# Strong-AI-Lab/ct-vae

Measured on AMD Instinct MI355X. Metric: images/sec/GPU fwd+bwd, 64×64×3 bs=64; recon+KL vs CPU ref, higher is better.
Workload: dtype f32; 1 GPU; VanillaVAE 64x64x3 train step fwd+loss+bwd+Adam (configs/vae.yaml shapes at the batch BASELINE.json's metric names, bs=64, on one MI355X; BASELINE.json configs[1..4] are the `configs` entries); per_gpu_batch=64, global_batch=64, latent_dim=128, parallelism=single, hipgraph=True, allreduce_overlap=False

## Files before the change

ct-vae_amd/csrc/api.hip:

```cpp
#include "../../include/ctvae_hip.h"

#include "common.hpp"
#include "gatlayer.hpp"
#include "glinear.hpp"
#include "pair.hpp"

namespace ctvae {
int launch_tapgemm(const ConvGeom& g, const float* G, const float* W, const float* bias, const float* add,
                   const float* mask, int mask_act, float* S, int act, float* bn_part, float* ws, size_t ws_floats,
                   hipStream_t st, const BnBwdFuse* bnb = nullptr, const InXform* xf = nullptr,
                   const WinoFilters* wf = nullptr, SplitKRaw* raw = nullptr, int out_pix = 0);
bool out_pix_supported(const ConvGeom& g, size_t ws_floats, int out_pix);
bool wino_supported(const ConvGeom& g, size_t ws_floats);
bool wino_enabled();
int wino_set_enabled(int on);
int launch_crop_resize_u8(const unsigned char* img, const long long* rows, float* out, int B, int N, int H, int W, int crop,
                          int S, hipStream_t st);
bool thin_forward_supported(const ConvGeom& g);
bool thin_wgrad_supported(const ConvGeom& g);
int tapgemm_bnb_rows(const ConvGeom& g, size_t ws_floats);
bool img_dgrad_supported(const ConvGeom& g);
void tapgemm_plan(const ConvGeom& g, size_t ws_floats, TapGemmPlan& p);
int launch_wgrad(const ConvGeom& g, const float* X, const float* dY, float* dW, float* dbias, float* ws, size_t ws_bytes,
                 int accumulate, hipStream_t st, const InXform* xf = nullptr, const DyXform* dyx = nullptr);
int launch_bn_forward(const float* y, int R, int C, const float* gamma, const float* beta, float* running_mean,
                      float* running_var, float momentum, float eps, int training, int act, float* out, float* save_mean,
                      float* save_invstd, float* ws, size_t ws_bytes, long long* nbt, hipStream_t st,
                      float* coef_out = nullptr);
int launch_bn_finish_forward(const float* y, int R, int C, int nparts, const float* gamma, const float* beta,
                             float* running_mean, float* running_var, float momentum, float eps, int training, int act,
                             float* out, float* save_mean, float* save_invstd, float* ws, long long* nbt, hipStream_t st,
                             float* coef_out = nullptr, const float* mean_base = nullptr);
size_t bn_workspace_floats(int C, int nparts);
int launch_bn_backward(const float* ga, const float* beta, const float* y, int R, int C, const float* gamma,
                       const float* save_mean, const float* save_invstd, int act, float* gy, float* dgamma, float* dbeta,
                       int accumulate, float* ws, size_t ws_bytes, const float* part_in, int part_rows, hipStream_t st,
                       float* coef_out = nullptr, const float* coef_in = nullptr);
int launch_wino_filters_batch(int n, const float* const* W, float* const* Uf, float* const* Ub, const int* Ci, const int* Co,
                              hipStream_t st);
bool upconv_wgrad_supported(const ConvGeom& g);
bool img_enc_supported(const ConvGeom& g);
bool img_conv_supported(const ConvGeom& g);
int launch_img_backward_fused(const ConvGeom& g, const float* dY, const float* W, float* dX, const BnBwdFuse* bnb, float* ws,
                              float** part_out, float** pbias_out, int* nparts, bool want_bias, hipStream_t st);
size_t img_backward_fused_ws_floats(const ConvGeom& g);
int wgrad_finish_slabs(const float* part, float* dW, long n, int nparts, const float* pbias, float* dbias, long nb, int accumulate,
                       hipStream_t st);
int launch_permute(const float* in, float* out, int B, int C, int P, int to_nhwc, hipStream_t st);
int launch_gat_score(int mode, const float* xl, const float* xr, const float* attr, const float* we, const float* att, float* out,
                     int B, int N, int H, int C, float slope, hipStream_t st);
int launch_gat_score_backward(const float* xl, const float* xr, const float* attr, const float* we, const float* att,
                              const float* g, float* dxl, float* dxr, float* datt_part, float* dwe_part, int B, int N, int H,
                              int C, float slope, hipStream_t st);
int launch_gauss_latent_fwd(float* heads, const float* eps_in, const unsigned long long* rng, float* eps_out, float* z, int B,
                            int L, hipStream_t st, const float* slices, int S, const float* bias);
int launch_splitk_permute(const float* slices, int S, float* out, int B, int C, int P, hipStream_t st);
int launch_gauss_latent_bwd(const float* g_mu, const float* g_lv, const float* g_z, const float* heads, const float* eps,
                            float* g_heads, unsigned long long* rng_bump, int B, int L, hipStream_t st, int gz_slices);
int launch_ct_reg_forward(const float* adj, const float* graph, const float* uni, float* part, float ckl, float cgs, float cpt,
                          int B, int N, hipStream_t st);
int launch_ct_reg_backward(const float* adj, const float* graph, const float* uni, const float* part, const float* g_loss,
                           float ckl, float cgs, float cpt, float* d_adj, float* d_graph, int B, int N, hipStream_t st);
int launch_ct_blend_softmax_forward(const float* y, const float* mask, float* probs, long R, int Hs, int D, hipStream_t st);
int launch_ct_blend_softmax_backward(const float* g, const float* probs, const float* y, const float* mask, float* dy, float* dmask,
                                     long R, int Hs, int D, hipStream_t st);
int launch_ct_latent_ce_forward(const float* probs, const long long* target, float* row_loss, long R, int D, hipStream_t st);
int launch_ct_latent_ce_backward(const float* probs, const long long* target, const float* g_loss, float* d_probs, long R, int D,
                                 hipStream_t st);
int launch_ct_mask_forward(const float* x, const float* action, const float* pe, const float* keep, float scale, const float* W,
                           const float* bias, const float* expo, int B, int S, int D, int A, float* inter, float* p, float* sample,
                           float* soft, hipStream_t st);
int launch_ct_mask_backward(const float* x, const float* action, const float* pe, const float* keep, float scale,
                            const float* inter, const float* p, const float* soft, const float* g, int B, int S, int D, int A,
                            float* dWp, float* dbp, hipStream_t st);
int launch_ladder_forward(const float* mu_e, const float* lv_e, const float* mu_t, const float* lv_t, const float* eps, int B, int D,
                          float* z, float* kl, hipStream_t st);
int launch_ladder_backward(const float* gz, const float* gkl, const float* mu_e, const float* lv_e, const float* mu_t, const float* lv_t,
                           const float* eps, int B, int D, float* g_mu_e, float* g_lv_e, float* g_mu_t, float* g_lv_t, hipStream_t st);
int launch_gamma_reparam_forward(const float* alpha, const float* beta, const float* zhat, float shape_b, float* z, long n, hipStream_t st);
int launch_gamma_reparam_backward(const float* g, const float* alpha, const float* beta, const float* zhat, float shape_b, float* ga,
                                  float* gb, long n, hipStream_t st);
int launch_gamma_kl_forward(const float* alpha, const float* beta, int B, int D, float prior_alpha, float prior_beta, float* out,
                            float* ws, size_t ws_bytes, hipStream_t st);
int launch_gamma_kl_backward(const float* g, const float* alpha, const float* beta, int B, int D, float prior_alpha, float prior_beta,
                             float* ga, float* gb, hipStream_t st);
int launch_sigmoid(const float* x_or_g, const float* y, float* out, long n, int backward, hipStream_t st);
int launch_tc_forward(const float* z, const float* mu, const float* lv, const float* liw, int B, int D, float* out3, float* lse_s,
                      float* lse_d, float* ws, size_t ws_bytes, hipStream_t st);
int launch_tc_backward(const float* z, const float* mu, const float* lv, const float* liw, const float* lse_s, const float* lse_d,
                       const float* g3, int B, int D, float* dz, float* dmu, float* dlv, hipStream_t st);
int launch_vamp_forward(const float* z, const float* mu, const float* lv, const float* pmu, const float* plv, int B, int D, int K,
                        float* out3, float* wgt, float* ws, size_t ws_bytes, hipStream_t st);
int launch_vamp_backward(const float* z, const float* mu, const float* lv, const float* pmu, const float* plv, const float* wgt,
                         const float* g, int B, int D, int K, float* dz, float* dmu, float* dlv, float* dpmu, float* dplv,
                         hipStream_t st);
int launch_swd_forward(const float* z, const float* prior, const float* proj, int N, int D, int S, float p, float weight, float* out,
                       float* grad_z, float* ws, size_t ws_bytes, hipStream_t st);
int launch_ct_blend_forward(const float* s0, const float* s1, const float* mask, float* out, long rows, hipStream_t st);
int launch_ct_blend_backward(const float* g, const float* s0, const float* s1, const float* mask, float* g0, float* g1, float* gm,
                             long rows, hipStream_t st);
int launch_group_rowsum(const float* parts, long mat_stride, int nmat, int rows, int C, int ld, const int* grp, int G, float* out,
                        int accumulate, hipStream_t st);
int launch_ct_posenc_forward(const float* x, const float* pe, const float* keep, float scale, float* out, long n, int sd,
                             hipStream_t st);
int launch_ct_posenc_backward(const float* g, const float* keep, float scale, float* gx, long n, hipStream_t st);
int launch_one_hot(const long long* inds, long n, int N, float* out, hipStream_t st);
int launch_ct_sample_forward(const float* p, const float* expo, float* out, float* soft, float* weighted, long n, hipStream_t st);
int launch_ct_sample_backward(const float* gs, const float* gw, const float* p, const float* soft, const float* sample, float* gp,
                              long n, hipStream_t st);
int launch_pair_mlp_forward(const float* u, const float* v, int ld, const float* w2, const float* b2, float* out, int B, int N,
                            int H, float slope, int per_sample, const int* row_of, hipStream_t st);
int launch_pair_mlp_backward(const float* u, const float* v, int ld, const float* w2, const float* out, const float* g_out,
                             float* dU, float* dV, int ldd, float* dw2_part, float* db2_part, int B, int N, int H, float slope,
                             int per_sample, const int* row_of, hipStream_t st);
int launch_act_bwd(const float* gout, const float* out, float* gin, long n, int act, hipStream_t st);
int launch_act_fwd(const float* in, float* out, long n, int act, hipStream_t st);
int launch_reparam_fwd(const float* mu, long mu_rs, const float* lv, long lv_rs, const float* eps, float* z, int B, int L,
                       hipStream_t st);
int launch_reparam_bwd(const float* gz, const float* lv, long lv_rs, const float* eps, float* gmu, float* glv, int B, int L,
                       hipStream_t st);
int launch_adam(float* p, const float* g, float* m, float* v, float* state, long n, float grad_scale, hipStream_t st);
size_t adam_state_floats();
int launch_adam_clipped(float* p, const float* g, float* m, float* v, float* state, long n, float grad_scale, int algorithm,
                        float clip, float* ws, float* norm_out, hipStream_t st);
size_t grad_clip_workspace_floats();
int launch_adam_mark_members(int* hits, int nhits, const int* group, int B, hipStream_t st);
int launch_adam_block_flags(const int* present, const int* hit_index, int* hits, int nhits, const float* bstate, int* active,
                            int nb, int until_first, hipStream_t st);
int launch_adam_block_flags_local(const int* present, const int* hit_index, int* hits, int nhits, int* active, int nb,
                                  hipStream_t st);
int launch_adam_block_flags_finish(const float* bstate, int* active, int nb, int until_first, hipStream_t st);
int launch_adam_blocks(float* p, const float* g, float* m, float* v, float* state, long n, float grad_scale, int algorithm,
                       float clip, float* ws, float* norm_out, const int* blk_lo, const int* blk_hi, float* bstate,
                       const int* active, int nb, hipStream_t st);
int launch_ssim_forward(const float* a, const float* b, const float* window, float* part, float* loss, float* coef, int B, int C, int H,
                        int W, const float* weights, hipStream_t st);
int launch_ssim_backward(const float* a, const float* b, const float* window, const float* coef, const float* g_loss, float* g_a, int B,
                         int C, int H, int W, hipStream_t st);
float* defer_wgrad_ws(float* ws, size_t ws_floats);
void defer_wgrad_done();
int defer_begin(float* arena, size_t arena_floats);
int defer_flush(hipStream_t st);
int launch_gumbel_fwd(const float* p, const float* noise, float* out, float* soft, long n, hipStream_t st);
int launch_gumbel_bwd(const float* go, const float* p, const float* soft, float* gp, long n, hipStream_t st);
int launch_gumbel_softmax_fwd(const float* z, const float* u, float* s, long rows, int Q, float temp, float eps, hipStream_t st);
int launch_gumbel_softmax_bwd(const float* gs, const float* s, float* gz, long rows, int Q, float temp, hipStream_t st);
int launch_cat_kl_fwd(const float* logits, long rows, int Q, int B, float eps, float c, float* out, float* ws, size_t ws_bytes,
                      hipStream_t st);
int launch_cat_kl_bwd(const float* logits, const float* go, float* gq, long rows, int Q, int B, float eps, float c, hipStream_t st);
int launch_iw_loss_forward(const float* recons, const float* x, long n, int R, int rep, const float* mu, const float* lv, int L,
                           int S, float M_N, float* lp, float* kld, float* coef, float* out4, hipStream_t st);
int launch_iw_loss_backward(const float* recons, const float* x, long n, int R, int rep, const float* mu, const float* lv, int L,
                            float M_N, const float* coef, const float* go, float* g_recons, float* g_mu, float* g_lv,
                            hipStream_t st);
int launch_mmd_forward(const float* z, const float* p, int N, int D, int kind, float c, float eps, float w_pp, float w_zz,
                       float w_pz, float* out4, float* grad, float* ws, size_t ws_bytes, hipStream_t st);
size_t dip_state_floats(int B, int D);
int launch_dip_forward(const float* mu, long mu_rs, const float* lv, long lv_rs, int B, int D, float l_diag, float l_off,
                       float* state, hipStream_t st);
int launch_dip_backward(const float* state, const float* go, float* g_mu, float* g_lv, int B, int D, hipStream_t st);
int launch_column_moments(const float* z, int N, int L, float* mean, float* var, float* mn, float* mx, hipStream_t st);
int launch_mi_matrix(const float* z, const float* lo, const float* hi, const int32_t* factors, const int32_t* sizes, int N, int L,
                     int F, float* mi, uint8_t* bins, hipStream_t st);
int launch_group_var_argmin(const float* z, const float* gvar, const uint8_t* active, int G, int B, int L, int32_t* arg, float* val,
                            hipStream_t st);
int launch_image_grid_u8(const float* x, long sN, long sC, long sH, long sW, int N, int C, int H, int W, int nrow, int pad,
                         int normalize, int has_range, float lo, float hi, float pad_value, int scanlines, uint8_t* out,
                         size_t out_bytes, float* ws, size_t ws_bytes, hipStream_t st);
int launch_image_grid_each_u8(const float* x, long sN, long sC, long sH, long sW, int N, int C, int H, int W, int nrow, int pad,
                              int normalize, int has_range, float lo, float hi, float pad_value, int scanlines, uint8_t* out,
                              size_t out_bytes, float* ws, size_t ws_bytes, hipStream_t st);
int launch_action_hits(const float* probas, const float* action, int N, int A, int* counts, hipStream_t st);
int launch_loss_forward(const float* r, const float* x, long n, const float* mu, long mu_rs, const float* lv, long lv_rs,
                        int B, int L, float M_N, const float* extra, float* out4, float* ws, size_t ws_bytes,
                        hipStream_t st, float logcosh_alpha, float* g_r = nullptr, float* g_mu = nullptr, float* g_lv = nullptr,
                        int ract = 0);
int launch_mse_backward(const float* r, const float* x, const float* go, float* gr, long n, hipStream_t st, float logcosh_alpha,
                        int ract = 0);
int launch_loss_backward(const float* r, const float* x, const float* go, float* gr, long n, float logcosh_alpha, const float* mu,
                         long mu_rs, const float* lv, long lv_rs, float* gmu, float* glv, int B, int L, float M_N, hipStream_t st,
                         int ract = 0);
int launch_kl_backward(const float* mu, long mu_rs, const float* lv, long lv_rs, const float* go, float* gmu, float* glv,
                       int B, int L, float M_N, hipStream_t st);
int launch_vq_inds(const float* lat, const float* cb, long long* inds, int B, int HW, int D, int K, int C, hipStream_t st);
int launch_vq_lookup(const float* lat, const float* cb, const long long* inds, float* out, float* vq_loss, float beta, int B,
                     int HW, int D, int K, int C, float* ws, size_t ws_bytes, hipStream_t st);
int launch_vq_backward(const float* gq, const float* gvq, const float* lat, const float* cb, const long long* inds,
                       float* glat, float* dcb, int accumulate, float beta, int B, int HW, int D, int K, int C, float* ws, size_t ws_bytes,
                       hipStream_t st);
}

using namespace ctvae;

static bool conv_kind_ok(int kind) {
  const int base = kind & ~CTVAE_W_CI_TAP;
  return base == CTVAE_CONV || (base == CTVAE_CONVT && !(kind & CTVAE_W_CI_TAP));
}
static int conv_geom(ConvGeom& g, int kind, int gkind0, int B, int H, int W, int Ci, int Co, int k, int stride, int pad, int out_pad) {
  const int rc = build_geom(g, gkind0 + ((kind & ~CTVAE_W_CI_TAP) == CTVAE_CONV ? 0 : 1), B, H, W, Ci, Co, k, stride, pad, out_pad);
  if (rc) return rc;
  if (kind & CTVAE_W_CI_TAP) {
    g.wts = Co;
    g.wrs = k * k * Co;
  }
  return 0;
}

extern "C" {

const char* ctvae_version(void) { return "0.1.0"; }
const char* ctvae_arch(void) { return "gfx950"; }

const char* ctvae_error_string(int code) {
  if (code == 0) return "success";
  if (code == kErrBadArg) return "ctvae: unsupported shape or bad argument";
  if (code == kErrWorkspace) return "ctvae: workspace too small";
  if (code > 0) return hipGetErrorString((hipError_t)code);
  return "ctvae: unknown error";
}

int ctvae_crop_resize_u8(const uint8_t* images, const int64_t* rows, float* out, int B, int N, int H, int W, int crop, int size,
                         void* stream) {
  if (!images || !rows || !out) return kErrBadArg;
  return launch_crop_resize_u8(images, (const long long*)rows, out, B, N, H, W, crop, size, (hipStream_t)stream);
}

int ctvae_winograd_enable(int on) { return wino_set_enabled(on); }

size_t ctvae_workspace_bytes(void) { return (size_t)256 << 20; }

int ctvae_conv_forward(int kind, const float* x, const float* w, const float* bias, const float* add, float* y, int B,
                       int H, int W, int Ci, int Co, int k, int stride, int pad, int out_pad, int act, const float* in_scale,
                       const float* in_shift, int in_act, float* wino_dgrad_filters_out, const float* wino_fwd_filters, float* ws,
                       size_t ws_bytes, void* stream) {
  if (!x || !w || !y || !conv_kind_ok(kind)) return kErrBadArg;
  if ((in_scale != nullptr) != (in_shift != nullptr)) return kErrBadArg;
  ConvGeom g;
  if (conv_geom(g, kind, 0, B, H, W, Ci, Co, k, stride, pad, out_pad)) return kErrBadArg;
  if ((wino_dgrad_filters_out != nullptr || wino_fwd_filters != nullptr) &&
      !ctvae_conv_wino_filter_floats(kind, B, H, W, Ci, Co, k, stride, pad, out_pad, ws_bytes))
    return kErrBadArg;
  const InXform xf{in_scale, in_shift, in_act};
  const WinoFilters wf{wino_fwd_filters, wino_fwd_filters != nullptr ? nullptr : wino_dgrad_filters_out};
  return launch_tapgemm(g, x, w, bias, add, nullptr, 0, y, act, nullptr, ws, ws_bytes / sizeof(float), (hipStream_t)stream,
                        nullptr, &xf, &wf);
}

int ctvae_linear_pixmajor_supported(int B, int Ci, int C, int P, size_t ws_bytes) {
  ConvGeom g;
  if (B <= 0 || Ci <= 0 || C <= 0 || P <= 1 || conv_geom(g, CTVAE_CONV, 0, B, 1, 1, Ci, C * P, 1, 1, 0, 0)) return 0;
  return out_pix_supported(g, ws_bytes / sizeof(float), P) ? 1 : 0;
}

int ctvae_linear_pixmajor_forward(const float* x, const float* w, const float* bias, float* y, int B, int Ci, int C, int P, int act,
                                  float* ws, size_t ws_bytes, void* stream) {
  if (!x || !w || !y || !ctvae_linear_pixmajor_supported(B, Ci, C, P, ws_bytes)) return kErrBadArg;
  ConvGeom g;
  if (conv_geom(g, CTVAE_CONV, 0, B, 1, 1, Ci, C * P, 1, 1, 0, 0)) return kErrBadArg;
  return launch_tapgemm(g, x, w, bias, nullptr, nullptr, 0, y, act, nullptr, ws, ws_bytes / sizeof(float), (hipStream_t)stream,
                        nullptr, nullptr, nullptr, nullptr, P);
}

int ctvae_wino_filters_batch(int n, const float* const* w, float* const* fwd_filters, float* const* dgrad_filters, const int* Ci,
                             const int* Co, void* stream) {
  return launch_wino_filters_batch(n, w, fwd_filters, dgrad_filters, Ci, Co, (hipStream_t)stream);
}

size_t ctvae_conv_wino_filter_floats(int kind, int B, int H, int W, int Ci, int Co, int k, int stride, int pad, int out_pad,
                                     size_t ws_bytes) {
  if (kind != CTVAE_CONV || !wino_enabled()) return 0;
  ConvGeom gf, gb;
  if (build_geom(gf, 0, B, H, W, Ci, Co, k, stride, pad, out_pad) || build_geom(gb, 2, B, H, W, Ci, Co, k, stride, pad, out_pad))
    return 0;
  const size_t wsf = ws_bytes / sizeof(float);
  return (wino_supported(gf, wsf) && wino_supported(gb, wsf)) ? (size_t)16 * Ci * Co : 0;
}

int ctvae_conv_input_transform_supported(int kind, int B, int H, int W, int Ci, int Co, int k, int stride, int pad,
                                         int out_pad) {
  if (!conv_kind_ok(kind)) return 0;
  ConvGeom g;
  if (conv_geom(g, kind, 0, B, H, W, Ci, Co, k, stride, pad, out_pad)) return 0;
  if (thin_forward_supported(g) && thin_wgrad_supported(g)) return 1;
  if (upconv_wgrad_supported(g)) return 1;
  if (img_enc_supported(g) || img_conv_supported(g)) return 0;
  if (wino_enabled() && wino_supported(g, (size_t)1 << 26)) return 0;
  TapGemmPlan pl;
  tapgemm_plan(g, (size_t)1 << 26, pl);
  if (pl.thin || pl.BM == 0) return 0;
  return ((g.gC % KC) == 0 && (g.sC % 4) == 0 && g.wT == 0) ? 1 : 0;
}

int ctvae_conv_bn_act_apply_is_separate(int kind, int B, int H, int W, int Ci, int Co, int k, int stride, int pad, int out_pad,
                                        size_t ws_bytes) {
  if (!conv_kind_ok(kind)) return 0;
  ConvGeom g;
  if (conv_geom(g, kind, 0, B, H, W, Ci, Co, k, stride, pad, out_pad)) return 0;
  TapGemmPlan plan;
  tapgemm_plan(g, ws_bytes / sizeof(float), plan);
  return (plan.splitk > 1 && bn_fused_ok(g.B * g.sH * g.sW, Co)) ? 0 : 1;
}

int ctvae_conv_bn_act_forward(int kind, const float* x, const float* w, const float* bias, const float* gamma,
                              const float* beta, float* running_mean, float* running_var, float momentum, float eps,
                              int training, int act, float* y, float* a_out, float* save_mean, float* save_invstd,
                              float* scale_shift_out, int64_t* num_batches_tracked, int B, int H, int W, int Ci, int Co, int k,
                              int stride, int pad, int out_pad, const float* in_scale, const float* in_shift, int in_act,
                              float* ws, size_t ws_bytes, void* stream) {
  long long* nbt = (long long*)num_batches_tracked;
  if (!x || !w || !gamma || !beta || !y || !ws || !conv_kind_ok(kind)) return kErrBadArg;
  if ((in_scale != nullptr) != (in_shift != nullptr)) return kErrBadArg;
  if (in_scale != nullptr && !ctvae_conv_input_transform_supported(kind, B, H, W, Ci, Co, k, stride, pad, out_pad)) return kErrBadArg;
  const InXform xf{in_scale, in_shift, in_act};
  const InXform* xfp = in_scale != nullptr ? &xf : nullptr;
  if (!a_out && !scale_shift_out) return kErrBadArg;
  if (training && (!save_mean || !save_invstd)) return kErrBadArg;
  if (!training && (!running_mean || !running_var)) return kErrBadArg;
  if (Co % 4 != 0) return kErrBadArg;
  ConvGeom g;
  if (conv_geom(g, kind, 0, B, H, W, Ci, Co, k, stride, pad, out_pad)) return kErrBadArg;
  const size_t wsf = ws_bytes / sizeof(float);
  TapGemmPlan plan;
  tapgemm_plan(g, wsf, plan);
  const int R = g.B * g.sH * g.sW;
  if (plan.splitk > 1 || !training) {
    SplitKRaw raw{ws, 0};
    const bool fused = training && plan.splitk > 1 && bn_fused_ok(R, Co);
    int rc = launch_tapgemm(g, x, w, bias, nullptr, nullptr, 0, y, ACT_NONE, nullptr, ws, wsf, (hipStream_t)stream, nullptr, xfp,
                            nullptr, fused ? &raw : nullptr);
    if (rc) return rc;
    if (raw.splitk > 1) {
      const BnFusedFwd p{ws, row_map_of(g), raw.splitk, R, Co, bias, gamma, beta, running_mean, running_var, momentum, eps, save_mean, save_invstd,
                         scale_shift_out, nbt, y, a_out, act};
      return launch_bn_fused_forward(p, (hipStream_t)stream);
    }
    return launch_bn_forward(y, R, Co, gamma, beta, running_mean, running_var, momentum, eps, training, act, a_out, save_mean,
                             save_invstd, ws, ws_bytes, nbt, (hipStream_t)stream, scale_shift_out);
  }
  const int nparts = plan.bn_parts;
  if (wsf < bn_workspace_floats(Co, nparts)) return kErrWorkspace;
  int rc = launch_tapgemm(g, x, w, bias, nullptr, nullptr, 0, y, ACT_NONE, ws, nullptr, 0, (hipStream_t)stream, nullptr, xfp);
  if (rc) return rc;
  return launch_bn_finish_forward(y, R, Co, nparts, gamma, beta, running_mean, running_var, momentum, eps, training, act,
                                  a_out, save_mean, save_invstd, ws, nbt, (hipStream_t)stream, scale_shift_out);
}

int ctvae_conv_dgrad(int kind, const float* dy, const float* w, const float* add, const float* mask, int mask_act,
                     float* dx, int B, int H, int W, int Ci, int Co, int k, int stride, int pad, int out_pad,
                     const float* wino_filters, float* ws, size_t ws_bytes, void* stream) {
  if (!dy || !w || !dx || !conv_kind_ok(kind)) return kErrBadArg;
  ConvGeom g;
  if (conv_geom(g, kind, 2, B, H, W, Ci, Co, k, stride, pad, out_pad)) return kErrBadArg;
  if (wino_filters != nullptr && !ctvae_conv_wino_filter_floats(kind, B, H, W, Ci, Co, k, stride, pad, out_pad, ws_bytes))
    return kErrBadArg;
  const WinoFilters wf{wino_filters, nullptr};
  return launch_tapgemm(g, dy, w, nullptr, add, mask, mask_act, dx, ACT_NONE, nullptr, ws, ws_bytes / sizeof(float),
                        (hipStream_t)stream, nullptr, nullptr, &wf);
}

int ctvae_conv_wgrad(int kind, const float* x, const float* dy, float* dw, float* dbias, int B, int H, int W, int Ci,
                     int Co, int k, int stride, int pad, int out_pad, int accumulate, const float* in_scale,
                     const float* in_shift, int in_act, const float* dy_bn_y, const float* dy_bn_coef, int dy_bn_act,
                     float* gy_out, float* bn_dgamma, float* bn_dbeta, int bn_accumulate, float* ws, size_t ws_bytes,
                     void* stream) {
  if (!x || !dy || !dw || !ws || !conv_kind_ok(kind)) return kErrBadArg;
  if ((in_scale != nullptr) != (in_shift != nullptr)) return kErrBadArg;
  if ((dy_bn_y != nullptr) != (dy_bn_coef != nullptr) || (gy_out != nullptr && dy_bn_y == nullptr)) return kErrBadArg;
  if ((bn_dgamma != nullptr) != (bn_dbeta != nullptr) || (bn_dgamma != nullptr && (dy_bn_y == nullptr || gy_out != nullptr)))
    return kErrBadArg;
  ConvGeom g;
  if (conv_geom(g, kind, 0, B, H, W, Ci, Co, k, stride, pad, out_pad)) return kErrBadArg;
  const InXform xf{in_scale, in_shift, in_act};
  const DyXform dyx{dy_bn_y, dy_bn_coef, gy_out, dy_bn_act, bn_dgamma, bn_dbeta, bn_accumulate};
  float* wws = defer_wgrad_ws(ws, ws_bytes / sizeof(float));
  const int rc = launch_wgrad(g, x, dy, dw, dbias, wws, ws_bytes, accumulate, (hipStream_t)stream, &xf, &dyx);
  defer_wgrad_done();
  return rc;
}

int ctvae_defer_begin(float* arena, size_t arena_bytes) { return defer_begin(arena, arena_bytes / sizeof(float)); }
int ctvae_defer_flush(void* stream) { return defer_flush((hipStream_t)stream); }

int ctvae_conv_backward_bn_rows(int kind, int B, int H, int W, int Ci, int Co, int k, int stride, int pad, int out_pad,
                                size_t ws_bytes) {
  if (!conv_kind_ok(kind)) return 0;
  ConvGeom g;
  if (conv_geom(g, kind, 2, B, H, W, Ci, Co, k, stride, pad, out_pad)) return 0;
  PairCtx ctx;
  pair_ctx() = &ctx;
  const int rows = tapgemm_bnb_rows(g, ((ws_bytes / 2) & ~(size_t)255) / sizeof(float));
  pair_ctx() = nullptr;
  return rows;
}

static thread_local int g_lazy_pixel_major = 0;

static int conv_backward_impl(int kind, const float* x, const float* dy, const float* w, float* dw, float* dbias, float* dx, int B,
                        int H, int W, int Ci, int Co, int k, int stride, int pad, int out_pad, int accumulate, const float* mask,
                        int mask_act, const float* wino_filters, const float* bn_y, const float* bn_mean,
                        const float* bn_invstd, const float* bn_gamma, const float* bn_beta, int bn_act, float* bn_part,
                        int bn_part_rows, float* bn_coef_out, float* bn_dgamma, float* bn_dbeta, int bn_accumulate,
                        const float* in_scale, const float* in_shift, int in_act,
                        const float* dy_bn_y, const float* dy_bn_coef, int dy_bn_act, float* gy_out, float* ws, size_t ws_bytes,
                        void* stream, float* dx_slices) {
  if (!x || !dy || !w || !dw || (!dx && !dx_slices) || !ws || !conv_kind_ok(kind)) return kErrBadArg;
  const bool bn = bn_part != nullptr;
  if (bn_coef_out != nullptr && !bn) return kErrBadArg;
  if ((bn_dgamma != nullptr) != (bn_dbeta != nullptr) || (bn_dgamma != nullptr && bn_coef_out == nullptr)) return kErrBadArg;
  if ((in_scale != nullptr) != (in_shift != nullptr)) return kErrBadArg;
  if ((dy_bn_y != nullptr) != (dy_bn_coef != nullptr) || (dy_bn_y != nullptr) != (gy_out != nullptr)) return kErrBadArg;
  if (bn && (!bn_y || !bn_mean || !bn_invstd || !bn_gamma || !bn_beta)) return kErrBadArg;
  ConvGeom gw, gd;
  if (conv_geom(gw, kind, 0, B, H, W, Ci, Co, k, stride, pad, out_pad)) return kErrBadArg;
  if (conv_geom(gd, kind, 2, B, H, W, Ci, Co, k, stride, pad, out_pad)) return kErrBadArg;
  const size_t half_bytes = (ws_bytes / 2) & ~(size_t)255, half_floats = half_bytes / sizeof(float);
  float* ws_d = ws + half_floats;
  if (wino_filters != nullptr && !ctvae_conv_wino_filter_floats(kind, B, H, W, Ci, Co, k, stride, pad, out_pad, half_bytes))
    return kErrBadArg;
  const hipStream_t st = (hipStream_t)stream;
  PairCtx ctx;
  pair_ctx() = &ctx;
  if (bn) {
    const int rows = tapgemm_bnb_rows(gd, half_floats);
    if (rows <= 0 || rows != bn_part_rows || (img_dgrad_supported(gd) && mask != nullptr)) {
      pair_ctx() = nullptr;
      return kErrBadArg;
    }
  }
  {
    TapGemmPlan pl;
    tapgemm_plan(gd, half_floats, pl);
    ctx.dgrad_wgs = (long)pl.mtiles * pl.ntiles * gd.ncls * (pl.splitk > 1 ? pl.splitk : 1);
    int kmax = 0;
    for (int c = 0; c < gd.ncls; ++c) kmax = gd.ntaps[c] * gd.gC / KC > kmax ? gd.ntaps[c] * gd.gC / KC : kmax;
    ctx.dgrad_chunks = pl.splitk > 1 ? (kmax + pl.splitk - 1) / pl.splitk : kmax;
  }
  const InXform xf{in_scale, in_shift, in_act};
  const DyXform dyx{dy_bn_y, dy_bn_coef, gy_out, dy_bn_act};
  int rc;
  if (bn && bn_act != ACT_TANH && x == bn_y && in_scale != nullptr && in_act == bn_act && mask == nullptr && dy_bn_y == nullptr &&
      img_conv_supported(gw) && img_dgrad_supported(gd) && img_backward_fused_ws_floats(gd) <= half_floats) {
    float *part = nullptr, *pb = nullptr;
    int np = 0;
    const BnBwdFuse f{bn_y, bn_mean, bn_invstd, bn_gamma, bn_beta, bn_act, bn_part};
    rc = launch_img_backward_fused(gd, dy, w, dx, &f, ws, &part, &pb, &np, dbias != nullptr, st);
    if (!rc) rc = wgrad_finish_slabs(part, dw, 9L * 32 * 3, np, pb, dbias, 3L, accumulate, st);
  } else {
    float* wws = bn_coef_out == nullptr ? defer_wgrad_ws(ws, half_floats) : ws;
    rc = launch_wgrad(gw, x, dy, dw, dbias, wws, half_bytes, accumulate, st, &xf, &dyx);
    defer_wgrad_done();
    if (!rc) {
    const WinoFilters wf{wino_filters, nullptr};
    const BnBwdFuse f{bn_y, bn_mean, bn_invstd, bn_gamma, bn_beta, bn_act, bn_part};
      SplitKRaw raw{dx_slices, 0, g_lazy_pixel_major};
      g_lazy_pixel_major = 0;
      rc = launch_tapgemm(gd, gy_out != nullptr ? gy_out : dy, w, nullptr, nullptr, mask, mask_act, dx, ACT_NONE, nullptr, ws_d,
                          half_floats, st, bn ? &f : nullptr, nullptr, &wf, dx_slices != nullptr ? &raw : nullptr);
      if (!rc && dx_slices != nullptr && raw.splitk <= 1) rc = kErrBadArg;
    }
  }
  pair_ctx() = nullptr;
  if (rc) return rc;
  if (bn_coef_out != nullptr) {
    ctx.haveBF = true;
    ctx.bf = BnFinJob{bn_part, bn_part_rows, Ci, (float)((long)B * H * W), bn_gamma, bn_mean, bn_invstd, bn_beta, bn_coef_out,
                      bn_dgamma, bn_dbeta, bn_accumulate};
  }
  return pair_flush(ctx, st);
}

int ctvae_conv_backward(int kind, const float* x, const float* dy, const float* w, float* dw, float* dbias, float* dx, int B,
                        int H, int W, int Ci, int Co, int k, int stride, int pad, int out_pad, int accumulate, const float* mask,
                        int mask_act, const float* wino_filters, const float* bn_y, const float* bn_mean,
                        const float* bn_invstd, const float* bn_gamma, const float* bn_beta, int bn_act, float* bn_part,
                        int bn_part_rows, float* bn_coef_out, float* bn_dgamma, float* bn_dbeta, int bn_accumulate,
                        const float* in_scale, const float* in_shift, int in_act,
                        const float* dy_bn_y, const float* dy_bn_coef, int dy_bn_act, float* gy_out, float* ws, size_t ws_bytes,
                        void* stream) {
  return conv_backward_impl(kind, x, dy, w, dw, dbias, dx, B, H, W, Ci, Co, k, stride, pad, out_pad, accumulate, mask, mask_act,
                            wino_filters, bn_y, bn_mean, bn_invstd, bn_gamma, bn_beta, bn_act, bn_part, bn_part_rows, bn_coef_out,
                            bn_dgamma, bn_dbeta, bn_accumulate, in_scale, in_shift, in_act, dy_bn_y, dy_bn_coef, dy_bn_act, gy_out, ws,
                            ws_bytes, stream, nullptr);
}

int ctvae_conv_backward_lazy_slices(int kind, int B, int H, int W, int Ci, int Co, int k, int stride, int pad, int out_pad,
                                    int for_bn, size_t ws_bytes) {
  if (!conv_kind_ok(kind)) return 0;
  ConvGeom g;
  if (conv_geom(g, kind, 2, B, H, W, Ci, Co, k, stride, pad, out_pad)) return 0;
  const size_t half_floats = ((ws_bytes / 2) & ~(size_t)255) / sizeof(float);
  if (img_dgrad_supported(g) || (wino_enabled() && wino_supported(g, half_floats))) return 0;
  PairCtx ctx;
  pair_ctx() = &ctx;
  TapGemmPlan pl;
  tapgemm_plan(g, half_floats, pl);
  pair_ctx() = nullptr;
  const long Mc = (long)g.B * g.Qh * g.Qw;
  if (pl.thin || pl.splitk <= 1) return 0;
  if (for_bn && (Mc % 4 != 0 || !bn_fused_ok(B * H * W, Ci))) return 0;
  return pl.splitk;
}

int ctvae_conv_backward_lazy(int kind, const float* x, const float* dy, const float* w, float* dw, float* dbias, float* dx_slices,
                             int B, int H, int W, int Ci, int Co, int k, int stride, int pad, int out_pad, int accumulate,
                             const float* in_scale, const float* in_shift, int in_act, int pixel_major, float* ws, size_t ws_bytes,
                             void* stream) {
  if (!dx_slices) return kErrBadArg;
  g_lazy_pixel_major = pixel_major;
  return conv_backward_impl(kind, x, dy, w, dw, dbias, nullptr, B, H, W, Ci, Co, k, stride, pad, out_pad, accumulate, nullptr, 0,
                            nullptr, nullptr, nullptr, nullptr, nullptr, nullptr, 0, nullptr, 0, nullptr, nullptr, nullptr, 0, in_scale,
                            in_shift, in_act, nullptr, nullptr, 0, nullptr, ws, ws_bytes, stream, dx_slices);
}

int ctvae_bn_backward_fused(const float* g_a_slices, int slices, int kind, int B, int H, int W, int Ci, int Co, int k, int stride,
                            int pad, int out_pad, const float* y, const float* gamma, const float* beta, const float* save_mean,
                            const float* save_invstd, int act, float* g_y, float* dgamma, float* dbeta, int accumulate, void* stream) {
  if (!g_a_slices || slices < 1 || !y || !gamma || !beta || !save_mean || !save_invstd || !g_y || !dgamma || !dbeta) return kErrBadArg;
  if (!conv_kind_ok(kind)) return kErrBadArg;
  ConvGeom g;
  if (conv_geom(g, kind, 2, B, H, W, Ci, Co, k, stride, pad, out_pad)) return kErrBadArg;
  const BnFusedBwd p{g_a_slices, row_map_of(g), slices, B * H * W, Ci, y, gamma, beta, save_mean, save_invstd, act, g_y, dgamma,
                     dbeta, accumulate};
  return launch_bn_fused_backward(p, (hipStream_t)stream);
}

int ctvae_conv_wgrad_bn_apply_supported(int kind, int B, int H, int W, int Ci, int Co, int k, int stride, int pad, int out_pad) {
  if (!conv_kind_ok(kind)) return 0;
  ConvGeom g;
  if (conv_geom(g, kind, 0, B, H, W, Ci, Co, k, stride, pad, out_pad)) return 0;
  if (upconv_wgrad_supported(g)) return 1;
  return img_enc_supported(g) ? 2 : 0;
}

int ctvae_bn_forward(const float* y, int R, int C, const float* gamma, const float* beta, float* running_mean,
                     float* running_var, float momentum, float eps, int training, int act, float* out,
                     float* save_mean, float* save_invstd, int64_t* num_batches_tracked, float* ws, size_t ws_bytes,
                     void* stream) {
  if (!y || !gamma || !beta || !out || !ws) return kErrBadArg;
  if (training && (!save_mean || !save_invstd)) return kErrBadArg;
  if (!training && (!running_mean || !running_var)) return kErrBadArg;
  return launch_bn_forward(y, R, C, gamma, beta, running_mean, running_var, momentum, eps, training, act, out, save_mean,
                           save_invstd, ws, ws_bytes, (long long*)num_batches_tracked, (hipStream_t)stream);
}

int ctvae_bn_backward(const float* g_a, const float* beta, const float* y, int R, int C, const float* gamma,
                      const float* save_mean, const float* save_invstd, int act, float* g_y, float* dgamma,
                      float* dbeta, int accumulate, const float* part_in, int part_rows, float* coef_out,
                      const float* coef_in, float* ws, size_t ws_bytes, void* stream) {
  if (!g_a || !beta || !y || !gamma || !save_mean || !save_invstd || !dgamma || !dbeta || !ws) return kErrBadArg;
  if (!g_y && !coef_out) return kErrBadArg;
  if ((part_in != nullptr) != (part_rows > 0)) return kErrBadArg;
  if (coef_in != nullptr && (!g_y || part_in != nullptr || coef_out != nullptr)) return kErrBadArg;
  return launch_bn_backward(g_a, beta, y, R, C, gamma, save_mean, save_invstd, act, g_y, dgamma, dbeta, accumulate, ws,
                            ws_bytes, part_in, part_rows, (hipStream_t)stream, coef_out, coef_in);
}

int ctvae_gat_score(int mode, const float* xl, const float* xr, const float* attr, const float* we, const float* att, float* out,
                    int B, int N, int H, int C, float slope, void* stream) {
  if (!xl || !xr || !attr || !we || !att || !out || (mode != 0 && mode != 1)) return kErrBadArg;
  return launch_gat_score(mode, xl, xr, attr, we, att, out, B, N, H, C, slope, (hipStream_t)stream);
}

int ctvae_gat_score_backward(const float* xl, const float* xr, const float* attr, const float* we, const float* att,
                             const float* g, float* d_xl, float* d_xr, float* d_att_part, float* d_we_part, int B, int N, int H,
                             int C, float slope, void* stream) {
  if (!xl || !xr || !attr || !we || !att || !g || !d_xl || !d_xr || !d_att_part || !d_we_part) return kErrBadArg;
  return launch_gat_score_backward(xl, xr, attr, we, att, g, d_xl, d_xr, d_att_part, d_we_part, B, N, H, C, slope,
                                   (hipStream_t)stream);
}

int ctvae_gat_layer_forward(const float* xl, const float* xr, int ld, const float* adj, const float* we, const float* att,
                            const float* bias, const int32_t* head_map, float* out, int ldo, float* alpha, int B, int Hs, int C,
                            float slope, int act, void* stream) {
  const GatLayerArgs a{xl, xr, ld, adj, we, att, bias, head_map, out, ldo, alpha, B, Hs, C, slope, act};
  return launch_gat_layer_forward(a, (hipStream_t)stream);
}

int ctvae_gat_layer_backward(const float* xl, const float* xr, int ld, const float* adj, const float* we, const float* att,
                             const float* bias, const int32_t* head_map, const float* out, int ldo, const float* alpha,
                             const float* g_out, float* dS, float* dattr, float* d_xl, float* d_xr, int ldd, float* d_bias_part,
                             float* d_att_part, float* d_we_part, float* d_adj, int accumulate_dadj, int B, int Hs, int C,
                             float slope, int act, void* stream) {
  GatBwdArgs p{};
  p.f = GatLayerArgs{xl, xr, ld, adj, we, att, bias, head_map, const_cast<float*>(out), ldo, const_cast<float*>(alpha), B, Hs, C,
                     slope, act};
  p.g_out = g_out; p.dS = dS; p.dattr = dattr; p.dxl = d_xl; p.dxr = d_xr; p.ldd = ldd;
  p.dbias_part = d_bias_part; p.datt_part = d_att_part; p.dwe_part = d_we_part;
  return launch_gat_layer_backward(p, d_adj, accumulate_dadj, (hipStream_t)stream);
}

int ctvae_gauss_latent_forward(float* heads, const float* eps_in, const uint64_t* rng, float* eps_out, float* z, int B, int L,
                               const float* head_slices, int slices, const float* head_bias, void* stream) {
  return launch_gauss_latent_fwd(heads, eps_in, (const unsigned long long*)rng, eps_out, z, B, L, (hipStream_t)stream, head_slices,
                                 slices, head_bias);
}

int ctvae_gauss_latent_backward(const float* g_mu, const float* g_logvar, const float* g_z, const float* heads, const float* eps,
                                float* g_heads, uint64_t* rng_bump, int B, int L, int g_z_slices, void* stream) {
  return launch_gauss_latent_bwd(g_mu, g_logvar, g_z, heads, eps, g_heads, (unsigned long long*)rng_bump, B, L, (hipStream_t)stream,
                                 g_z_slices);
}

int ctvae_splitk_permute(const float* slices, int n_slices, float* out, int B, int C, int P, void* stream) {
  return launch_splitk_permute(slices, n_slices, out, B, C, P, (hipStream_t)stream);
}

int ctvae_conv_forward_lazy_slices(int kind, int B, int H, int W, int Ci, int Co, int k, int stride, int pad, int out_pad,
                                   size_t ws_bytes) {
  if (!conv_kind_ok(kind)) return 0;
  ConvGeom g;
  if (conv_geom(g, kind, 0, B, H, W, Ci, Co, k, stride, pad, out_pad)) return 0;
  const size_t wsf = ws_bytes / sizeof(float);
  if (img_enc_supported(g) || img_conv_supported(g) || upconv_wgrad_supported(g) || (wino_enabled() && wino_supported(g, wsf))) return 0;
  TapGemmPlan pl;
  tapgemm_plan(g, wsf, pl);
  return (pl.thin || pl.splitk <= 1) ? 0 : pl.splitk;
}

int ctvae_conv_forward_lazy(int kind, const float* x, const float* w, float* y_slices, int B, int H, int W, int Ci, int Co, int k,
                            int stride, int pad, int out_pad, float* ws, size_t ws_bytes, void* stream) {
  if (!x || !w || !y_slices || !ws || !conv_kind_ok(kind)) return kErrBadArg;
  ConvGeom g;
  if (conv_geom(g, kind, 0, B, H, W, Ci, Co, k, stride, pad, out_pad)) return kErrBadArg;
  SplitKRaw raw{y_slices, 0, 1};
  const int rc = launch_tapgemm(g, x, w, nullptr, nullptr, nullptr, 0, nullptr, ACT_NONE, nullptr, ws, ws_bytes / sizeof(float),
                                (hipStream_t)stream, nullptr, nullptr, nullptr, &raw);
  if (rc) return rc;
  return raw.splitk > 1 ? 0 : kErrBadArg;
}

int ctvae_ct_reg_forward(const float* adj, const float* graph, const float* uniform, float* part4, float ckl, float cgs, float cpt,
                         int B, int N, void* stream) {
  return launch_ct_reg_forward(adj, graph, uniform, part4, ckl, cgs, cpt, B, N, (hipStream_t)stream);
}

int ctvae_ct_reg_backward(const float* adj, const float* graph, const float* uniform, const float* part4, const float* g_loss,
                          float ckl, float cgs, float cpt, float* d_adj, float* d_graph, int B, int N, void* stream) {
  return launch_ct_reg_backward(adj, graph, uniform, part4, g_loss, ckl, cgs, cpt, d_adj, d_graph, B, N, (hipStream_t)stream);
}

int ctvae_ct_blend_softmax_forward(const float* y, const float* mask, float* probs, long R, int Hs, int D, void* stream) {
  return launch_ct_blend_softmax_forward(y, mask, probs, R, Hs, D, (hipStream_t)stream);
}

int ctvae_ct_blend_softmax_backward(const float* g, const float* probs, const float* y, const float* mask, float* dy, float* dmask,
                                    long R, int Hs, int D, void* stream) {
  return launch_ct_blend_softmax_backward(g, probs, y, mask, dy, dmask, R, Hs, D, (hipStream_t)stream);
}

int ctvae_ct_latent_ce_forward(const float* probs, const int64_t* target, float* row_loss, long R, int D, void* stream) {
  return launch_ct_latent_ce_forward(probs, (const long long*)target, row_loss, R, D, (hipStream_t)stream);
}

int ctvae_ct_latent_ce_backward(const float* probs, const int64_t* target, const float* g_loss, float* d_probs, long R, int D,
                                void* stream) {
  return launch_ct_latent_ce_backward(probs, (const long long*)target, g_loss, d_probs, R, D, (hipStream_t)stream);
}

int ctvae_ct_mask_forward(const float* x, const float* action, const float* pe, const float* keep, float scale, const float* W,
                          const float* bias, const float* expo, int B, int S, int D, int A, float* inter, float* p, float* sample,
                          float* soft, void* stream) {
  return launch_ct_mask_forward(x, action, pe, keep, scale, W, bias, expo, B, S, D, A, inter, p, sample, soft, (hipStream_t)stream);
}

int ctvae_ct_mask_backward(const float* x, const float* action, const float* pe, const float* keep, float scale, const float* inter,
                           const float* p, const float* soft, const float* g, int B, int S, int D, int A, float* dWp, float* dbp,
                           void* stream) {
  return launch_ct_mask_backward(x, action, pe, keep, scale, inter, p, soft, g, B, S, D, A, dWp, dbp, (hipStream_t)stream);
}

int ctvae_ct_sample_forward(const float* p, const float* expo, float* sample, float* soft, float* weighted, long n, void* stream) {
  return launch_ct_sample_forward(p, expo, sample, soft, weighted, n, (hipStream_t)stream);
}

int ctvae_ct_sample_backward(const float* g_sample, const float* g_weighted, const float* p, const float* soft, const float* sample,
                             float* g_p, long n, void* stream) {
  return launch_ct_sample_backward(g_sample, g_weighted, p, soft, sample, g_p, n, (hipStream_t)stream);
}

int ctvae_ct_blend_forward(const float* s0, const float* s1, const float* mask, float* out, long rows, void* stream) {
  return launch_ct_blend_forward(s0, s1, mask, out, rows, (hipStream_t)stream);
}

int ctvae_ct_blend_backward(const float* g, const float* s0, const float* s1, const float* mask, float* g0, float* g1, float* g_mask,
                            long rows, void* stream) {
  return launch_ct_blend_backward(g, s0, s1, mask, g0, g1, g_mask, rows, (hipStream_t)stream);
}

int ctvae_ct_posenc_forward(const float* x, const float* pe, const float* keep, float scale, float* out, long n, int sd,
                            void* stream) {
  return launch_ct_posenc_forward(x, pe, keep, scale, out, n, sd, (hipStream_t)stream);
}

int ctvae_ct_posenc_backward(const float* g, const float* keep, float scale, float* g_x, long n, void* stream) {
  return launch_ct_posenc_backward(g, keep, scale, g_x, n, (hipStream_t)stream);
}

int ctvae_one_hot(const int64_t* inds, long n, int N, float* out, void* stream) {
  return launch_one_hot((const long long*)inds, n, N, out, (hipStream_t)stream);
}

int ctvae_group_rowsum(const float* parts, long mat_stride, int nmat, int rows, int C, int ld, const int32_t* group, int G, float* out,
                       int accumulate, void* stream) {
  return launch_group_rowsum(parts, mat_stride, nmat, rows, C, ld, group, G, out, accumulate, (hipStream_t)stream);
}

static int glin_fill(GLinArgs& a, int nseg, int N, const float* const* W, const int* ldw, const int64_t* w_gstride,
                     const float* const* bias, const int* b_gstride, const int32_t* const* group) {
  if (nseg < 1 || nseg > kGLinMaxSeg || !W || !ldw || !w_gstride) return kErrBadArg;
  a.nseg = nseg;
  a.N = N;
  for (int s = 0; s < nseg; ++s) {
    a.W[s] = W[s];
    a.ldw[s] = ldw[s];
    a.wgs[s] = (long)w_gstride[s];
    a.bias[s] = bias ? bias[s] : nullptr;
    a.bgs[s] = b_gstride ? b_gstride[s] : 0;
    a.group[s] = group ? group[s] : nullptr;
  }
  return 0;
}

int ctvae_glinear_forward(const float* x, int ldx, int K, int nseg, int N, const float* const* W, const int* ldw,
                          const int64_t* w_gstride, const float* const* bias, const int* b_gstride,
                          const int32_t* const* group, float* y, int ldy, int B, void* stream) {
  GLinArgs a{};
  if (int rc = glin_fill(a, nseg, N, W, ldw, w_gstride, bias, b_gstride, group)) return rc;
  a.x = x; a.ldx = ldx; a.K = K; a.y = y; a.ldy = ldy; a.B = B;
  return launch_glinear_forward(a, (hipStream_t)stream);
}

int ctvae_glinear_dgrad(const float* dy, int ldy, int nseg, int N, const float* const* W, const int* ldw,
                        const int64_t* w_gstride, const int32_t* const* group, float* dx, int ldx, int K, int B, void* stream) {
  GLinArgs a{};
  if (int rc = glin_fill(a, nseg, N, W, ldw, w_gstride, nullptr, nullptr, group)) return rc;
  a.x = nullptr; a.ldx = ldx; a.K = K; a.y = const_cast<float*>(dy); a.ldy = ldy; a.B = B;
  return launch_glinear_dgrad(a, dx, (hipStream_t)stream);
}

size_t ctvae_glinear_wgrad_ws_bytes(int G, int N, int K, int B, int grouped) {
  if (G <= 0 || N <= 0 || K <= 0 || B <= 0) return 0;
  return glinear_wgrad_ws_floats(G, N, K, glinear_wgrad_slices(B, G, grouped != 0)) * sizeof(float);
}

int ctvae_glinear_wgrad(const float* x, int ldx, int K, const float* dy, int ldy, int col0, int N, const int32_t* group, int G,
                        int B, float* dW, int ldo, float* dbias, int accumulate, float* ws, size_t ws_bytes, void* stream) {
  return launch_glinear_wgrad(x, ldx, K, dy, ldy, col0, N, group, G, B, dW, ldo, dbias, accumulate, ws, ws_bytes / sizeof(float),
                              (hipStream_t)stream);
}

int ctvae_pair_mlp_forward(const float* u, const float* v, int ld, const float* w2, const float* b2, float* out, int B, int N,
                           int H, float slope, int per_sample, const int32_t* row_of, void* stream) {
  if (!u || !v || !w2 || !out) return kErrBadArg;
  return launch_pair_mlp_forward(u, v, ld, w2, b2, out, B, N, H, slope, per_sample, row_of, (hipStream_t)stream);
}

int ctvae_pair_mlp_backward(const float* u, const float* v, int ld, const float* w2, const float* out, const float* g_out,
                            float* d_u, float* d_v, int ldd, float* d_w2_part, float* d_b2_part, int B, int N, int H, float slope,
                            int per_sample, const int32_t* row_of, void* stream) {
  if (!u || !v || !w2 || !out || !g_out || !d_u || !d_v || !d_w2_part || !d_b2_part) return kErrBadArg;
  return launch_pair_mlp_backward(u, v, ld, w2, out, g_out, d_u, d_v, ldd, d_w2_part, d_b2_part, B, N, H, slope, per_sample,
                                  row_of, (hipStream_t)stream);
}

int ctvae_permute(const float* in, float* out, int B, int C, int P, int to_nhwc, void* stream) {
  if (!in || !out || B <= 0 || C <= 0 || P <= 0) return kErrBadArg;
  return launch_permute(in, out, B, C, P, to_nhwc, (hipStream_t)stream);
}

int ctvae_act_forward(const float* in, float* out, long n, int act, void* stream) {
  if (!in || !out || n <= 0) return kErrBadArg;
  return launch_act_fwd(in, out, n, act, (hipStream_t)stream);
}

int ctvae_act_backward(const float* g_out, const float* out, float* g_in, long n, int act, void* stream) {
  if (!g_out || !out || !g_in || n <= 0) return kErrBadArg;
  return launch_act_bwd(g_out, out, g_in, n, act, (hipStream_t)stream);
}

int ctvae_reparam_forward(const float* mu, long mu_rs, const float* logvar, long lv_rs, const float* eps, float* z, int B,
                          int L, void* stream) {
  if (!mu || !logvar || !eps || !z || B <= 0 || L <= 0) return kErrBadArg;
  return launch_reparam_fwd(mu, mu_rs, logvar, lv_rs, eps, z, B, L, (hipStream_t)stream);
}

int ctvae_reparam_backward(const float* g_z, const float* logvar, long lv_rs, const float* eps, float* g_mu,
                           float* g_logvar, int B, int L, void* stream) {
  if (!g_z || !logvar || !eps || !g_mu || !g_logvar || B <= 0 || L <= 0) return kErrBadArg;
  return launch_reparam_bwd(g_z, logvar, lv_rs, eps, g_mu, g_logvar, B, L, (hipStream_t)stream);
}

int ctvae_loss_forward(const float* recons, const float* x, long n, const float* mu, long mu_rs, const float* logvar,
                       long lv_rs, int B, int L, float M_N, const float* extra, float* out4, float* ws, size_t ws_bytes,
                       void* stream) {
  if (!recons || !x || !out4 || !ws || n <= 0) return kErrBadArg;
  if ((mu == nullptr) != (logvar == nullptr)) return kErrBadArg;
  return launch_loss_forward(recons, x, n, mu, mu_rs, logvar, lv_rs, B, L, M_N, extra, out4, ws, ws_bytes,
                             (hipStream_t)stream, 0.f);
}

int ctvae_loss_forward_grad(const float* recons, const float* x, long n, const float* mu, long mu_rs, const float* logvar,
                            long lv_rs, int B, int L, float M_N, const float* extra, float* out4, float* g_recons, float* g_mu,
                            float* g_logvar, int recons_act, float* ws, size_t ws_bytes, void* stream) {
  if (!recons || !x || !out4 || !ws || n <= 0 || !mu || !logvar || !g_recons || !g_mu || !g_logvar) return kErrBadArg;
  return launch_loss_forward(recons, x, n, mu, mu_rs, logvar, lv_rs, B, L, M_N, extra, out4, ws, ws_bytes,
                             (hipStream_t)stream, 0.f, g_recons, g_mu, g_logvar, recons_act);
}

int ctvae_mse_backward(const float* recons, const float* x, const float* g_loss, float* g_recons, long n, int recons_act,
                       void* stream) {
  if (!recons || !x || !g_loss || !g_recons || n <= 0) return kErrBadArg;
  return launch_mse_backward(recons, x, g_loss, g_recons, n, (hipStream_t)stream, 0.f, recons_act);
}

int ctvae_loss_backward(const float* recons, const float* x, const float* g_loss, float* g_recons, long n, float logcosh_alpha,
                        const float* mu, long mu_rs, const float* logvar, long lv_rs, float* g_mu, float* g_logvar, int B, int L,
                        float M_N, int recons_act, void* stream) {
  if (!recons || !x || !g_loss || !g_recons || n <= 0 || !mu || !logvar || !g_mu || !g_logvar || B <= 0 || L <= 0) return kErrBadArg;
  return launch_loss_backward(recons, x, g_loss, g_recons, n, logcosh_alpha, mu, mu_rs, logvar, lv_rs, g_mu, g_logvar, B, L, M_N,
                              (hipStream_t)stream, recons_act);
}

int ctvae_l2l1_loss_forward(const float* recons, const float* x, long n, const float* extra, float* out4, float* ws, size_t ws_bytes,
                            void* stream) {
  if (!recons || !x || !out4 || !ws || n <= 0) return kErrBadArg;
  return launch_loss_forward(recons, x, n, nullptr, 0, nullptr, 0, 0, 0, 0.f, extra, out4, ws, ws_bytes, (hipStream_t)stream, -1.f);
}

int ctvae_l2l1_backward(const float* recons, const float* x, const float* g_loss, float* g_recons, long n, int recons_act,
                        void* stream) {
  if (!recons || !x || !g_loss || !g_recons || n <= 0) return kErrBadArg;
  return launch_mse_backward(recons, x, g_loss, g_recons, n, (hipStream_t)stream, -1.f, recons_act);
}

int ctvae_ladder_merge_forward(const float* mu_e, const float* logvar_e, const float* mu_t, const float* logvar_t, const float* eps,
                               int B, int D, float* z, float* kl, void* stream) {
  return launch_ladder_forward(mu_e, logvar_e, mu_t, logvar_t, eps, B, D, z, kl, (hipStream_t)stream);
}

int ctvae_ladder_merge_backward(const float* g_z, const float* g_kl, const float* mu_e, const float* logvar_e, const float* mu_t,
                                const float* logvar_t, const float* eps, int B, int D, float* g_mu_e, float* g_logvar_e,
                                float* g_mu_t, float* g_logvar_t, void* stream) {
  return launch_ladder_backward(g_z, g_kl, mu_e, logvar_e, mu_t, logvar_t, eps, B, D, g_mu_e, g_logvar_e, g_mu_t, g_logvar_t,
                                (hipStream_t)stream);
}

int ctvae_gamma_reparam_forward(const float* alpha, const float* beta, const float* zhat, float gamma_shape, float* z, long n,
                                void* stream) {
  return launch_gamma_reparam_forward(alpha, beta, zhat, gamma_shape, z, n, (hipStream_t)stream);
}

int ctvae_gamma_reparam_backward(const float* g_z, const float* alpha, const float* beta, const float* zhat, float gamma_shape,
                                 float* g_alpha, float* g_beta, long n, void* stream) {
  return launch_gamma_reparam_backward(g_z, alpha, beta, zhat, gamma_shape, g_alpha, g_beta, n, (hipStream_t)stream);
}

int ctvae_gamma_kl_forward(const float* alpha, const float* beta, int B, int D, float prior_alpha, float prior_beta, float* out,
                           float* ws, size_t ws_bytes, void* stream) {
  return launch_gamma_kl_forward(alpha, beta, B, D, prior_alpha, prior_beta, out, ws, ws_bytes, (hipStream_t)stream);
}

int ctvae_gamma_kl_backward(const float* g_kld, const float* alpha, const float* beta, int B, int D, float prior_alpha,
                            float prior_beta, float* g_alpha, float* g_beta, void* stream) {
  return launch_gamma_kl_backward(g_kld, alpha, beta, B, D, prior_alpha, prior_beta, g_alpha, g_beta, (hipStream_t)stream);
}

int ctvae_sigmoid_forward(const float* x, float* y, long n, void* stream) { return launch_sigmoid(x, nullptr, y, n, 0, (hipStream_t)stream); }

int ctvae_sigmoid_backward(const float* g, const float* y, float* g_x, long n, void* stream) {
  return launch_sigmoid(g, y, g_x, n, 1, (hipStream_t)stream);
}

int ctvae_tc_forward(const float* z, const float* mu, const float* logvar, const float* log_iw, int B, int D, float* out3, float* lse_s,
                     float* lse_d, float* ws, size_t ws_bytes, void* stream) {
  return launch_tc_forward(z, mu, logvar, log_iw, B, D, out3, lse_s, lse_d, ws, ws_bytes, (hipStream_t)stream);
}

int ctvae_tc_backward(const float* z, const float* mu, const float* logvar, const float* log_iw, const float* lse_s, const float* lse_d,
                      const float* g3, int B, int D, float* g_z, float* g_mu, float* g_logvar, void* stream) {
  return launch_tc_backward(z, mu, logvar, log_iw, lse_s, lse_d, g3, B, D, g_z, g_mu, g_logvar, (hipStream_t)stream);
}

int ctvae_vamp_kl_forward(const float* z, const float* mu, const float* logvar, const float* prior_mu, const float* prior_logvar,
                          int B, int D, int K, float* out3, float* weights, float* ws, size_t ws_bytes, void* stream) {
  return launch_vamp_forward(z, mu, logvar, prior_mu, prior_logvar, B, D, K, out3, weights, ws, ws_bytes, (hipStream_t)stream);
}

int ctvae_vamp_kl_backward(const float* z, const float* mu, const float* logvar, const float* prior_mu, const float* prior_logvar,
                           const float* weights, const float* g_kld, int B, int D, int K, float* g_z, float* g_mu, float* g_logvar,
                           float* g_prior_mu, float* g_prior_logvar, void* stream) {
  return launch_vamp_backward(z, mu, logvar, prior_mu, prior_logvar, weights, g_kld, B, D, K, g_z, g_mu, g_logvar, g_prior_mu,
                              g_prior_logvar, (hipStream_t)stream);
}

int ctvae_swd_forward(const float* z, const float* prior, const float* proj, int N, int D, int S, float p, float weight, float* out,
                      float* grad_z, float* ws, size_t ws_bytes, void* stream) {
  return launch_swd_forward(z, prior, proj, N, D, S, p, weight, out, grad_z, ws, ws_bytes, (hipStream_t)stream);
}

int ctvae_logcosh_loss_forward(const float* recons, const float* x, long n, float alpha, const float* mu, long mu_rs,
                               const float* logvar, long lv_rs, int B, int L, float M_N, float* out4, float* ws,
                               size_t ws_bytes, void* stream) {
  if (!recons || !x || !out4 || !ws || n <= 0 || !(alpha > 0.f)) return kErrBadArg;
  if ((mu == nullptr) != (logvar == nullptr)) return kErrBadArg;
  return launch_loss_forward(recons, x, n, mu, mu_rs, logvar, lv_rs, B, L, M_N, nullptr, out4, ws, ws_bytes,
                             (hipStream_t)stream, alpha);
}

int ctvae_logcosh_backward(const float* recons, const float* x, const float* g_loss, float* g_recons, long n, float alpha,
                           int recons_act, void* stream) {
  if (!recons || !x || !g_loss || !g_recons || n <= 0 || !(alpha > 0.f)) return kErrBadArg;
  return launch_mse_backward(recons, x, g_loss, g_recons, n, (hipStream_t)stream, alpha, recons_act);
}

int ctvae_kl_backward(const float* mu, long mu_rs, const float* logvar, long lv_rs, const float* g_loss, float* g_mu,
                      float* g_logvar, int B, int L, float M_N, void* stream) {
  if (!mu || !logvar || !g_loss || !g_mu || !g_logvar) return kErrBadArg;
  return launch_kl_backward(mu, mu_rs, logvar, lv_rs, g_loss, g_mu, g_logvar, B, L, M_N, (hipStream_t)stream);
}

int ctvae_vq_inds(const float* latents, const float* codebooks, int64_t* inds, int B, int HW, int D, int K, int C,
                  void* stream) {
  if (!latents || !codebooks || !inds || B <= 0 || HW <= 0 || C <= 0) return kErrBadArg;
  return launch_vq_inds(latents, codebooks, (long long*)inds, B, HW, D, K, C, (hipStream_t)stream);
}

int ctvae_vq_lookup(const float* latents, const float* codebooks, const int64_t* inds, float* quantized, float* vq_loss,
                    float beta, int B, int HW, int D, int K, int C, float* ws, size_t ws_bytes, void* stream) {
  if (!latents || !codebooks || !inds || !quantized || !vq_loss || !ws || C <= 0) return kErrBadArg;
  return launch_vq_lookup(latents, codebooks, (const long long*)inds, quantized, vq_loss, beta, B, HW, D, K, C, ws, ws_bytes,
                          (hipStream_t)stream);
}

int ctvae_vq_backward(const float* g_quantized, const float* g_vq_loss, const float* latents, const float* codebooks,
                      const int64_t* inds, float* g_latents, float* d_codebooks, int accumulate, float beta, int B, int HW,
                      int D, int K, int C, float* ws, size_t ws_bytes, void* stream) {
  if (!latents || !codebooks || !inds || C <= 0) return kErrBadArg;
  return launch_vq_backward(g_quantized, g_vq_loss, latents, codebooks, (const long long*)inds, g_latents, d_codebooks,
                            accumulate, beta, B, HW, D, K, C, ws, ws_bytes, (hipStream_t)stream);
}

int ctvae_gumbel_st_forward(const float* p, const float* gumbel_noise, float* sample, float* soft, long n, void* stream) {
  if (!p || !gumbel_noise || !sample || !soft || n <= 0) return kErrBadArg;
  return launch_gumbel_fwd(p, gumbel_noise, sample, soft, n, (hipStream_t)stream);
}

int ctvae_gumbel_st_backward(const float* g_sample, const float* p, const float* soft, float* g_p, long n, void* stream) {
  if (!g_sample || !p || !soft || !g_p || n <= 0) return kErrBadArg;
  return launch_gumbel_bwd(g_sample, p, soft, g_p, n, (hipStream_t)stream);
}

int ctvae_gumbel_softmax_forward(const float* logits, const float* uniform, float* sample, long rows, int Q, float temperature,
                                 float eps, void* stream) {
  if (!logits || !uniform || !sample || rows <= 0 || Q <= 0 || !(temperature > 0.f)) return kErrBadArg;
  return launch_gumbel_softmax_fwd(logits, uniform, sample, rows, Q, temperature, eps, (hipStream_t)stream);
}

int ctvae_gumbel_softmax_backward(const float* g_sample, const float* sample, float* g_logits, long rows, int Q,
                                  float temperature, void* stream) {
  if (!g_sample || !sample || !g_logits || rows <= 0 || Q <= 0 || !(temperature > 0.f)) return kErrBadArg;
  return launch_gumbel_softmax_bwd(g_sample, sample, g_logits, rows, Q, temperature, (hipStream_t)stream);
}

int ctvae_cat_kl_forward(const float* logits, long rows, int Q, int B, float eps, float log_prior, float* kld, float* ws,
                         size_t ws_bytes, void* stream) {
  if (!logits || !kld || !ws || rows <= 0 || Q <= 0 || B <= 0) return kErrBadArg;
  return launch_cat_kl_fwd(logits, rows, Q, B, eps, log_prior, kld, ws, ws_bytes, (hipStream_t)stream);
}

int ctvae_cat_kl_backward(const float* logits, const float* g_kld, float* g_logits, long rows, int Q, int B, float eps,
                          float log_prior, void* stream) {
  if (!logits || !g_kld || !g_logits || rows <= 0 || Q <= 0 || B <= 0) return kErrBadArg;
  return launch_cat_kl_bwd(logits, g_kld, g_logits, rows, Q, B, eps, log_prior, (hipStream_t)stream);
}

int ctvae_iw_loss_forward(const float* recons, const float* x, long n, int R, int rep, const float* mu, const float* logvar,
                          int L, int S, float M_N, float* lp, float* kld, float* coef, float* out4, void* stream) {
  if (!recons || !x || !mu || !logvar || !lp || !kld || !coef || !out4) return kErrBadArg;
  if (n <= 0 || (n & 3) || R <= 0 || rep <= 0 || R % rep || S <= 0 || R % S || L <= 0) return kErrBadArg;
  return launch_iw_loss_forward(recons, x, n, R, rep, mu, logvar, L, S, M_N, lp, kld, coef, out4, (hipStream_t)stream);
}

int ctvae_iw_loss_backward(const float* recons, const float* x, long n, int R, int rep, const float* mu, const float* logvar,
                           int L, float M_N, const float* coef, const float* g_loss, float* g_recons, float* g_mu,
                           float* g_logvar, void* stream) {
  if (!recons || !x || !mu || !logvar || !coef || !g_loss || (g_mu == nullptr) != (g_logvar == nullptr)) return kErrBadArg;
  if (n <= 0 || (n & 3) || R <= 0 || rep <= 0 || R % rep || L <= 0) return kErrBadArg;
  return launch_iw_loss_backward(recons, x, n, R, rep, mu, logvar, L, M_N, coef, g_loss, g_recons, g_mu, g_logvar,
                                 (hipStream_t)stream);
}

int ctvae_mmd_forward(const float* z, const float* prior, int N, int D, int kind, float c, float eps, float w_pp, float w_zz,
                      float w_pz, float* out4, float* grad_z, float* ws, size_t ws_bytes, void* stream) {
  if (!z || !prior || !out4 || !grad_z || !ws || N <= 0 || D <= 0 || (kind != 0 && kind != 1) || !(c > 0.f)) return kErrBadArg;
  return launch_mmd_forward(z, prior, N, D, kind, c, eps, w_pp, w_zz, w_pz, out4, grad_z, ws, ws_bytes, (hipStream_t)stream);
}

size_t ctvae_dip_state_floats(int B, int D) { return dip_state_floats(B, D); }

int ctvae_dip_forward(const float* mu, long mu_rs, const float* logvar, long lv_rs, int B, int D, float lambda_diag,
                      float lambda_offdiag, float* state, void* stream) {
  if (!mu || !logvar || !state || B <= 0 || D <= 0) return kErrBadArg;
  return launch_dip_forward(mu, mu_rs, logvar, lv_rs, B, D, lambda_diag, lambda_offdiag, state, (hipStream_t)stream);
}

int ctvae_dip_backward(const float* state, const float* g_dip, float* g_mu, float* g_logvar, int B, int D, void* stream) {
  if (!state || !g_dip || !g_mu || !g_logvar || B <= 0 || D <= 0) return kErrBadArg;
  return launch_dip_backward(state, g_dip, g_mu, g_logvar, B, D, (hipStream_t)stream);
}

int ctvae_column_moments(const float* z, int N, int L, float* mean, float* var, float* min, float* max, void* stream) {
  if (!z || !mean || !var || !min || !max) return kErrBadArg;
  return launch_column_moments(z, N, L, mean, var, min, max, (hipStream_t)stream);
}

int ctvae_mi_matrix(const float* z, const float* lo, const float* hi, const int32_t* factors, const int32_t* sizes, int N, int L,
                    int F, float* mi, uint8_t* bins, void* stream) {
  if (!z || !lo || !hi || !factors || !sizes || !mi) return kErrBadArg;
  return launch_mi_matrix(z, lo, hi, factors, sizes, N, L, F, mi, bins, (hipStream_t)stream);
}

int ctvae_group_var_argmin(const float* z, const float* global_var, const uint8_t* active, int G, int B, int L, int32_t* arg,
                           float* val, void* stream) {
  if (!z || !global_var || !active || !arg || !val) return kErrBadArg;
  return launch_group_var_argmin(z, global_var, active, G, B, L, arg, val, (hipStream_t)stream);
}

int ctvae_image_grid_u8(const float* x, long stride_n, long stride_c, long stride_h, long stride_w, int N, int C, int H, int W,
                        int nrow, int padding, int normalize, int has_range, float range_lo, float range_hi, float pad_value,
                        int scanlines, uint8_t* out, size_t out_bytes, float* workspace, size_t workspace_bytes, void* stream) {
  return launch_image_grid_u8(x, stride_n, stride_c, stride_h, stride_w, N, C, H, W, nrow, padding, normalize, has_range, range_lo,
                              range_hi, pad_value, scanlines, out, out_bytes, workspace, workspace_bytes, (hipStream_t)stream);
}

int ctvae_image_grid_each_u8(const float* x, long stride_n, long stride_c, long stride_h, long stride_w, int N, int C, int H, int W,
                             int nrow, int padding, int normalize, int has_range, float range_lo, float range_hi, float pad_value,
                             int scanlines, uint8_t* out, size_t out_bytes, float* workspace, size_t workspace_bytes, void* stream) {
  return launch_image_grid_each_u8(x, stride_n, stride_c, stride_h, stride_w, N, C, H, W, nrow, padding, normalize, has_range,
                                   range_lo, range_hi, pad_value, scanlines, out, out_bytes, workspace, workspace_bytes,
                                   (hipStream_t)stream);
}

int ctvae_action_hits(const float* probas, const float* action, int N, int A, int* counts, void* stream) {
  return launch_action_hits(probas, action, N, A, counts, (hipStream_t)stream);
}

size_t ctvae_adam_state_floats(void) { return adam_state_floats(); }

size_t ctvae_mssim_part_floats(int B, int C) { return (size_t)5 * B * C * 2; }
int ctvae_mssim_forward(const float* a, const float* b, const float* window, const float* weights, float* part, float* loss,
                        float* coef, int B, int C, int H, int W, void* stream) {
  return launch_ssim_forward(a, b, window, part, loss, coef, B, C, H, W, weights, (hipStream_t)stream);
}
int ctvae_mssim_backward(const float* a, const float* b, const float* window, const float* coef, const float* g_loss, float* g_a,
                         int B, int C, int H, int W, void* stream) {
  return launch_ssim_backward(a, b, window, coef, g_loss, g_a, B, C, H, W, (hipStream_t)stream);
}

int ctvae_adam_step(float* params, const float* grads, float* exp_avg, float* exp_avg_sq, float* state, long n,
                    float grad_scale, void* stream) {
  if (!params || !grads || !exp_avg || !exp_avg_sq || !state || n <= 0) return kErrBadArg;
  return launch_adam(params, grads, exp_avg, exp_avg_sq, state, n, grad_scale, (hipStream_t)stream);
}

size_t ctvae_grad_clip_workspace_floats(void) { return grad_clip_workspace_floats(); }

int ctvae_adam_step_clipped(float* params, const float* grads, float* exp_avg, float* exp_avg_sq, float* state, long n,
                            float grad_scale, int algorithm, float clip_val, float* workspace, float* norm_out, void* stream) {
  if (!params || !grads || !exp_avg || !exp_avg_sq || !state || n <= 0 || !(clip_val > 0.f)) return kErrBadArg;
  if (algorithm != CTVAE_CLIP_NORM && algorithm != CTVAE_CLIP_VALUE) return kErrBadArg;
  if (algorithm == CTVAE_CLIP_NORM && !workspace) return kErrBadArg;
  return launch_adam_clipped(params, grads, exp_avg, exp_avg_sq, state, n, grad_scale, algorithm, clip_val, workspace, norm_out,
                             (hipStream_t)stream);
}

int ctvae_adam_mark_members(int* hits, int nhits, const int* group, int B, void* stream) {
  if (!hits || nhits < 1 || B < 0 || (B > 0 && !group)) return kErrBadArg;
  return launch_adam_mark_members(hits, nhits, B > 0 ? group : nullptr, B, (hipStream_t)stream);
}

int ctvae_adam_block_flags(const int* present, const int* hit_index, int* hits, int nhits, const float* block_state, int* active,
                           int nb, int until_first, void* stream) {
  if (!present || !hit_index || !block_state || !active || nb < 1 || nhits < 0 || (nhits > 0 && !hits)) return kErrBadArg;
  return launch_adam_block_flags(present, hit_index, hits, nhits, block_state, active, nb, until_first, (hipStream_t)stream);
}

int ctvae_adam_block_flags_local(const int* present, const int* hit_index, int* hits, int nhits, int* active, int nb, void* stream) {
  if (!present || !hit_index || !active || nb < 1 || nhits < 0 || (nhits > 0 && !hits)) return kErrBadArg;
  return launch_adam_block_flags_local(present, hit_index, hits, nhits, active, nb, (hipStream_t)stream);
}

int ctvae_adam_block_flags_finish(const float* block_state, int* active, int nb, int until_first, void* stream) {
  if (!block_state || !active || nb < 1) return kErrBadArg;
  return launch_adam_block_flags_finish(block_state, active, nb, until_first, (hipStream_t)stream);
}

int ctvae_adam_step_blocks(float* params, const float* grads, float* exp_avg, float* exp_avg_sq, float* state, long n,
                           float grad_scale, int algorithm, float clip_val, float* workspace, float* norm_out,
                           const int* block_lo, const int* block_hi, float* block_state, const int* active, int nb, void* stream) {
  if (!params || !grads || !exp_avg || !exp_avg_sq || !state || n <= 0) return kErrBadArg;
  if (!block_lo || !block_hi || !block_state || !active || nb < 1) return kErrBadArg;
  if (algorithm != CTVAE_CLIP_NORM && algorithm != CTVAE_CLIP_VALUE && algorithm != CTVAE_ADAM_NO_CLIP) return kErrBadArg;
  if (algorithm != CTVAE_ADAM_NO_CLIP && !(clip_val > 0.f)) return kErrBadArg;
  if (algorithm == CTVAE_CLIP_NORM && !workspace) return kErrBadArg;
  return launch_adam_blocks(params, grads, exp_avg, exp_avg_sq, state, n, grad_scale, algorithm, clip_val, workspace, norm_out,
                            block_lo, block_hi, block_state, active, nb, (hipStream_t)stream);
}

}
```

ct-vae_amd/csrc/upconv.hip:

```cpp
#include "common.hpp"
#include "phase.hpp"
#include <type_traits>

#include "prof.hpp"

namespace ctvae {

namespace {

constexpr int TH = 8, TW = 32, PH = 9, PW = 33, NP = PH * PW ;
constexpr int LDA = 36, C = 32, NT = 9, NCLS = 4, MAXT = 4;
constexpr int NLD = (NP * 8 + 255) / 256;
constexpr unsigned kOOBu = 0x80000000u;

struct UpArgs {
  const float* X;
  const float* Wt;
  const float* bias;
  const float* dY;
  float* out;
  float* pbias;
  float* bn_part;
  const float* dy_y;
  const float* dy_coef;
  float* gy_out;
  int dy_act;
  const float* xf_scale;
  const float* xf_shift;
  int xf_act;
  int act;
  int B, H, W, tiles_y, tiles_x, ntiles;
  int ntaps[NCLS], cpy[NCLS], cpx[NCLS];
  int tdy[NCLS][MAXT], tdx[NCLS][MAXT], twt[NCLS][MAXT];
};

__device__ __forceinline__ f32x4 ld4(__amdgpu_buffer_rsrc_t r, unsigned off) {
  return __builtin_bit_cast(f32x4, __builtin_amdgcn_raw_buffer_load_b128(r, (int)off, 0, 0));
}
__device__ __forceinline__ float ld1(__amdgpu_buffer_rsrc_t r, unsigned off) {
  return __builtin_bit_cast(float, __builtin_amdgcn_raw_buffer_load_b32(r, (int)off, 0, 0));
}
__device__ __forceinline__ void st1(__amdgpu_buffer_rsrc_t r, unsigned off, float v) {
  __builtin_amdgcn_raw_buffer_store_b32(__builtin_bit_cast(unsigned, v), r, (int)off, 0, 0);
}
__device__ __forceinline__ __amdgpu_buffer_rsrc_t rsrc(const void* p, long bytes) {
  return __builtin_amdgcn_make_buffer_rsrc(const_cast<void*>(p), 0, (int)bytes, 0x00020000);
}

struct TileXY {
  int b, y0, x0;
};
__device__ __forceinline__ TileXY tile_xy(const UpArgs& a, int tile) {
  const int per = a.tiles_y * a.tiles_x;
  const int b = tile / per, r = tile - b * per;
  const int ty = r / a.tiles_x;
  return TileXY{b, ty * TH, (r - ty * a.tiles_x) * TW};
}

struct Patch {
  f32x4 v[NLD];
};
__device__ __forceinline__ void patch_load(const UpArgs& a, __amdgpu_buffer_rsrc_t rX, const TileXY& t, Patch& p) {
#pragma unroll
  for (int j = 0; j < NLD; ++j) {
    const int e = threadIdx.x + 256 * j;
    const int pp = e >> 3, c4 = e & 7;
    const int py = (pp * 1986) >> 16, px = pp - py * PW;
    const int iy = t.y0 + py, ix = t.x0 + px;
    const bool ok = e < NP * 8 && iy < a.H && ix < a.W;
    p.v[j] = ld4(rX, ok ? (unsigned)(((t.b * a.H + iy) * a.W + ix) * C + 4 * c4) * 4u : kOOBu);
  }
}
__device__ __forceinline__ void patch_store(const Patch& p, float* sA) {
#pragma unroll
  for (int j = 0; j < NLD; ++j) {
    const int e = threadIdx.x + 256 * j;
    if (e < NP * 8) *reinterpret_cast<f32x4*>(&sA[(e >> 3) * LDA + 4 * (e & 7)]) = p.v[j];
  }
}
__device__ __forceinline__ void patch_store_xf(const UpArgs& a, const TileXY& t, const Patch& p, float* sA, f32x4 sc, f32x4 sh,
                                               float nslope) {
#pragma unroll
  for (int j = 0; j < NLD; ++j) {
    const int e = threadIdx.x + 256 * j;
    const int pp = e >> 3;
    const int py = (pp * 1986) >> 16, px = pp - py * PW;
    const float inside = (t.y0 + py < a.H && t.x0 + px < a.W) ? 1.f : 0.f;
    f32x4 v = p.v[j];
#pragma unroll
    for (int q = 0; q < 4; ++q) {
      const float u = v[q] * sc[q] + sh[q] * inside;
      v[q] = fmaxf(u, u * nslope);
    }
    if (e < NP * 8) *reinterpret_cast<f32x4*>(&sA[pp * LDA + 4 * (e & 7)]) = v;
  }
}

CTVAE_PHASE_DECL(up)
__global__ __launch_bounds__(256, 2) void up_fwd_kernel(const UpArgs a) {
  CTVAE_PH(up, 0, 0);
  kernarg_warm<sizeof(UpArgs)>();
  extern __shared__ __attribute__((aligned(16))) float smem[];
  float* sA = smem;
  float* sW = smem + NP * LDA;
  __shared__ float sS[4 * C * 3];
  const int tid = threadIdx.x, lane = tid & 63, wave = tid >> 6, li = lane & 31, lh = lane >> 5;
  const __amdgpu_buffer_rsrc_t rX = rsrc(a.X, (long)a.B * a.H * a.W * C * 4);
  const int OH = 2 * a.H, OW = 2 * a.W;
  const __amdgpu_buffer_rsrc_t rO = rsrc(a.out, (long)a.B * OH * OW * C * 4);

  constexpr int NW4 = NT * C * C / 4 / 256;
  static_assert(NW4 * 256 * 4 == NT * C * C, "weights: a whole number of 16-byte loads per thread");
  f32x4 wv[NW4];
#pragma unroll
  for (int j = 0; j < NW4; ++j) wv[j] = reinterpret_cast<const f32x4*>(a.Wt)[tid + 256 * j];
  Patch pt;
  int tile = blockIdx.x;
  TileXY cur = tile_xy(a, tile < a.ntiles ? tile : 0);
  if (tile < a.ntiles) patch_load(a, rX, cur, pt);
  const float bv = a.bias != nullptr ? a.bias[li] : 0.f;
  const float out_slope = a.act == ACT_LRELU ? kLeaky : (a.act == ACT_RELU ? 0.f : 1.f);
  float sn = 0.f, smean = 0.f, sm2 = 0.f;

  const bool xf = a.xf_scale != nullptr;
  const f32x4 xsc = xf ? *reinterpret_cast<const f32x4*>(a.xf_scale + 4 * (tid & 7)) : f32x4{0.f, 0.f, 0.f, 0.f};
  const f32x4 xsh = xf ? *reinterpret_cast<const f32x4*>(a.xf_shift + 4 * (tid & 7)) : f32x4{0.f, 0.f, 0.f, 0.f};
  const float xns = a.xf_act == ACT_LRELU ? kLeaky : (a.xf_act == ACT_RELU ? 0.f : 1.f);
#pragma unroll
  for (int j = 0; j < NW4; ++j) reinterpret_cast<f32x4*>(sW)[tid + 256 * j] = wv[j];
  for (; tile < a.ntiles; tile += gridDim.x) {
    CTVAE_PH(up, 0, 1);
    if (xf) patch_store_xf(a, cur, pt, sA, xsc, xsh, xns);
    else patch_store(pt, sA);
    __syncthreads();
    CTVAE_PH(up, 0, 2);
    const int next = tile + gridDim.x;
    const TileXY nxt = tile_xy(a, next < a.ntiles ? next : 0);
    if (next < a.ntiles) patch_load(a, rX, nxt, pt);
    struct Frag {
      f32x4 af[4];
      float bf[4][4];
    };
    auto read_tap = [&](int ly, int c, int t, Frag& f) {
      const float* ap = &sA[((ly + a.tdy[c][t]) * PW + li + a.tdx[c][t]) * LDA + 4 * lh];
      const float* wp = &sW[(a.twt[c][t] * C + 4 * lh) * C + li];
#pragma unroll
      for (int kg = 0; kg < 4; ++kg) {
        f.af[kg] = *reinterpret_cast<const f32x4*>(ap + kg * 8);
#pragma unroll
        for (int q = 0; q < 4; ++q) f.bf[kg][q] = wp[(kg * 8 + q) * C];
      }
    };
    auto mfma_tap = [&](const Frag& f, f32x16& acc) {
#pragma unroll
      for (int kg = 0; kg < 4; ++kg)
#pragma unroll
        for (int q = 0; q < 4; ++q) acc = __builtin_amdgcn_mfma_f32_32x32x2f32(f.af[kg][q], f.bf[kg][q], acc, 0, 0, 0);
    };
    auto epilogue = [&](int ly, int c, f32x16& acc) {
      const unsigned rowoff = (unsigned)((((cur.b * OH + 2 * (cur.y0 + ly) + a.cpy[c]) * OW + 2 * cur.x0 + a.cpx[c]) * C + li)) * 4u;
      float m1 = 0.f;
      if (a.act == ACT_TANH) {
#pragma unroll
        for (int r = 0; r < 16; ++r) {
          acc[r] += bv;
          m1 += acc[r];
          st1(rO, rowoff + (unsigned)((8 * (r >> 2) + 4 * lh + (r & 3)) * 2 * C) * 4u, act_fwd(acc[r], ACT_TANH));
        }
      } else {
#pragma unroll
        for (int r = 0; r < 16; ++r) {
          acc[r] += bv;
          m1 += acc[r];
          st1(rO, rowoff + (unsigned)((8 * (r >> 2) + 4 * lh + (r & 3)) * 2 * C) * 4u, fmaxf(acc[r], acc[r] * out_slope));
        }
      }
      if (a.bn_part != nullptr) {
        m1 *= (1.f / 16.f);
        float q = 0.f;
#pragma unroll
        for (int r = 0; r < 16; ++r) q += (acc[r] - m1) * (acc[r] - m1);
        const float ntot = sn + 16.f, d = m1 - smean;
        smean += d * (16.f / ntot);
        sm2 += q + d * d * (sn * 16.f / ntot);
        sn = ntot;
      }
    };
    auto zero = [](f32x16& acc) {
#pragma unroll
      for (int r = 0; r < 16; ++r) acc[r] = 0.f;
    };
#define UP_STEP(LY, C_, T_, CUR, NXT, NLY, NC, NT_, HAS_NEXT)          \
    if (HAS_NEXT) read_tap(NLY, NC, NT_, NXT);                          \
    mfma_tap(CUR, acc);                                                 \
    _Pragma("unroll") for (int g_ = 0; g_ < 16; ++g_) {                 \
      __builtin_amdgcn_sched_group_barrier(0x008, 1, 0);                \
      __builtin_amdgcn_sched_group_barrier(0x100, 2, 0);                \
    }                                                                   \
    __builtin_amdgcn_sched_barrier(0);
    Frag fa, fb;
#pragma unroll 1
    for (int i = 0; i < 2; ++i) {
      const int ly = wave + 4 * i;
      f32x16 acc;
      read_tap(ly, 0, 0, fa);
      zero(acc);
      UP_STEP(ly, 0, 0, fa, fb, ly, 1, 0, true)
      epilogue(ly, 0, acc);
      zero(acc);
      UP_STEP(ly, 1, 0, fb, fa, ly, 1, 1, true)
      UP_STEP(ly, 1, 1, fa, fb, ly, 2, 0, true)
      epilogue(ly, 1, acc);
      zero(acc);
      UP_STEP(ly, 2, 0, fb, fa, ly, 2, 1, true)
      UP_STEP(ly, 2, 1, fa, fb, ly, 3, 0, true)
      epilogue(ly, 2, acc);
      zero(acc);
      UP_STEP(ly, 3, 0, fb, fa, ly, 3, 1, true)
      UP_STEP(ly, 3, 1, fa, fb, ly, 3, 2, true)
      UP_STEP(ly, 3, 2, fb, fa, ly, 3, 3, true)
      UP_STEP(ly, 3, 3, fa, fb, ly, 0, 0, false)
      epilogue(ly, 3, acc);
    }
#undef UP_STEP
    CTVAE_PH(up, 0, 3);
    __syncthreads();
    CTVAE_PH(up, 0, 4);
    cur = nxt;
  }
  if (a.bn_part != nullptr) {
    {
      const float on = __shfl_xor(sn, 32, 64), om = __shfl_xor(smean, 32, 64), oq = __shfl_xor(sm2, 32, 64);
      const float ntot = sn + on;
      if (ntot > 0.f) {
        const float d = om - smean;
        sm2 = sm2 + oq + d * d * (sn * on / ntot);
        smean = smean + d * (on / ntot);
      }
      sn = ntot;
    }
    if (lh == 0) {
      float* st = &sS[(wave * C + li) * 3];
      st[0] = sn; st[1] = smean; st[2] = sm2;
    }
    __syncthreads();
    if (tid < C) {
      float n = 0.f, mean = 0.f, m2 = 0.f;
#pragma unroll
      for (int w = 0; w < 4; ++w) {
        const float nb = sS[(w * C + tid) * 3], mb = sS[(w * C + tid) * 3 + 1], qb = sS[(w * C + tid) * 3 + 2];
        if (nb > 0.f) {
          const float ntot = n + nb, d = mb - mean;
          mean += d * (nb / ntot);
          m2 += qb + d * d * (n * nb / ntot);
          n = ntot;
        }
      }
      float* p = a.bn_part + ((long)blockIdx.x * C + tid) * 3;
      p[0] = n; p[1] = mean; p[2] = m2;
    }
  }
}


template <int CLS>
struct ClsInfo {
  static constexpr int ntaps = CLS == 0 ? 1 : (CLS == 3 ? 4 : 2);
  static constexpr int first = CLS == 0 ? 0 : (CLS == 1 ? 1 : (CLS == 2 ? 3 : 5));
};

template <bool FUSED>
__global__ __launch_bounds__(256, 1) void up_wgrad_kernel(const UpArgs a) {
  kernarg_warm<sizeof(UpArgs)>();
  __shared__ __attribute__((aligned(16))) float sA[NP * LDA];
  __shared__ __attribute__((aligned(16))) float sR[4 * C * C];
  __shared__ float sB[4 * C];
  const int tid = threadIdx.x, lane = tid & 63, wave = tid >> 6, li = lane & 31, lh = lane >> 5;
  const __amdgpu_buffer_rsrc_t rX = rsrc(a.X, (long)a.B * a.H * a.W * C * 4);
  const int OH = 2 * a.H, OW = 2 * a.W;
  const long obytes = (long)a.B * OH * OW * C * 4;
  const __amdgpu_buffer_rsrc_t rG = rsrc(a.dY, obytes);
  const __amdgpu_buffer_rsrc_t rYb = rsrc(a.dy_y, FUSED ? obytes : 0);
  const __amdgpu_buffer_rsrc_t rGY = rsrc(a.gy_out, FUSED ? obytes : 0);
  const float k1 = FUSED ? a.dy_coef[li] : 0.f, k2 = FUSED ? a.dy_coef[C + li] : 0.f, k3 = FUSED ? a.dy_coef[2 * C + li] : 0.f;
  const float ksc = FUSED ? a.dy_coef[3 * C + li] : 0.f, ksh = FUSED ? a.dy_coef[4 * C + li] : 0.f;
  const float nslope = a.dy_act == ACT_LRELU ? kLeaky : (a.dy_act == ACT_RELU ? 0.f : 1.f);
  const bool xf = a.xf_scale != nullptr;
  const f32x4 xsc = xf ? *reinterpret_cast<const f32x4*>(a.xf_scale + 4 * (tid & 7)) : f32x4{0.f, 0.f, 0.f, 0.f};
  const f32x4 xsh = xf ? *reinterpret_cast<const f32x4*>(a.xf_shift + 4 * (tid & 7)) : f32x4{0.f, 0.f, 0.f, 0.f};
  const float xns = a.xf_act == ACT_LRELU ? kLeaky : (a.xf_act == ACT_RELU ? 0.f : 1.f);

  f32x16 acc[NT];
#pragma unroll
  for (int t = 0; t < NT; ++t)
#pragma unroll
    for (int r = 0; r < 16; ++r) acc[t][r] = 0.f;
  float bsum = 0.f;

  CTVAE_PH(up, 1, 0);
  for (int tile = blockIdx.x; tile < a.ntiles; tile += gridDim.x) {
    const TileXY cur = tile_xy(a, tile);
    CTVAE_PH(up, 1, 1);
#pragma unroll
    for (int h = 0; h < 2; ++h) {
      f32x4 v[NLD / 2];
#pragma unroll
      for (int j = 0; j < NLD / 2; ++j) {
        const int e = tid + 256 * (j + h * (NLD / 2));
        const int pp = e >> 3, c4 = e & 7;
        const int py = (pp * 1986) >> 16, px = pp - py * PW;
        const int iy = cur.y0 + py, ix = cur.x0 + px;
        const bool ok = e < NP * 8 && iy < a.H && ix < a.W;
        v[j] = ld4(rX, ok ? (unsigned)(((cur.b * a.H + iy) * a.W + ix) * C + 4 * c4) * 4u : kOOBu);
      }
      if (xf) {
#pragma unroll
        for (int j = 0; j < NLD / 2; ++j) {
          const int e = tid + 256 * (j + h * (NLD / 2));
          const int pp = e >> 3;
          const int py = (pp * 1986) >> 16, px = pp - py * PW;
          const float inside = (cur.y0 + py < a.H && cur.x0 + px < a.W) ? 1.f : 0.f;
#pragma unroll
          for (int q = 0; q < 4; ++q) {
            const float u = v[j][q] * xsc[q] + xsh[q] * inside;
            v[j][q] = fmaxf(u, u * xns);
          }
        }
      }
#pragma unroll
      for (int j = 0; j < NLD / 2; ++j) {
        const int e = tid + 256 * (j + h * (NLD / 2));
        if (e < NP * 8) *reinterpret_cast<f32x4*>(&sA[(e >> 3) * LDA + 4 * (e & 7)]) = v[j];
      }
    }
    __syncthreads();

    CTVAE_PH(up, 1, 2);
    float dv[3][8], yv[FUSED ? 3 : 1][FUSED ? 8 : 1];
    auto step_off = [&](int ly, int c, int h) {
      return (unsigned)((((cur.b * OH + 2 * (cur.y0 + ly) + a.cpy[c]) * OW + 2 * cur.x0 + a.cpx[c] + 2 * (16 * h + lh)) * C + li)) * 4u;
    };
    auto dy_load = [&](unsigned off, auto slot_c) {
      constexpr int slot = decltype(slot_c)::value;
#pragma unroll
      for (int j = 0; j < 8; ++j) dv[slot][j] = ld1(rG, off + (unsigned)(4 * j * C) * 4u);
      if constexpr (FUSED) {
#pragma unroll
        for (int j = 0; j < 8; ++j) yv[slot][j] = ld1(rYb, off + (unsigned)(4 * j * C) * 4u);
      }
    };
    auto run_step = [&](int ly, auto cls_c, int h, unsigned off, auto slot_c) {
      constexpr int CLS = decltype(cls_c)::value;
      constexpr int slot = decltype(slot_c)::value;
      using CI = ClsInfo<CLS>;
      int xo[CI::ntaps];
#pragma unroll
      for (int t = 0; t < CI::ntaps; ++t) xo[t] = ((ly + a.tdy[CLS][t]) * PW + 16 * h + lh + a.tdx[CLS][t]) * LDA + li;
      float xa[CI::ntaps], xb[CI::ntaps];
#pragma unroll
      for (int t = 0; t < CI::ntaps; ++t) xa[t] = sA[xo[t]];
#pragma unroll
      for (int j = 0; j < 8; ++j) {
        if (j + 1 < 8) {
#pragma unroll
          for (int t = 0; t < CI::ntaps; ++t) xb[t] = sA[xo[t] + 2 * (j + 1) * LDA];
        }
        float d = dv[slot][j];
        if constexpr (FUSED) {
          const float yy = yv[slot][j];
          const float g1 = (yy * ksc + ksh) > 0.f ? d : d * nslope;
          d = k1 * g1 + k2 * yy + k3;
          st1(rGY, off + (unsigned)(4 * j * C) * 4u, d);
        }
        bsum += d;
#pragma unroll
        for (int t = 0; t < CI::ntaps; ++t)
          acc[CI::first + t] = __builtin_amdgcn_mfma_f32_32x32x2f32(xa[t], d, acc[CI::first + t], 0, 0, 0);
#pragma unroll
        for (int t = 0; t < CI::ntaps; ++t) xa[t] = xb[t];
        __builtin_amdgcn_sched_barrier(0);
      }
    };
    unsigned soff[3];
    auto issue = [&](auto s_c) {
      constexpr int S = decltype(s_c)::value;
      soff[S % 3] = step_off(wave + 4 * (S / 8), (S % 8) / 2, S & 1);
      dy_load(soff[S % 3], std::integral_constant<int, S % 3>{});
    };
    auto do_step = [&](auto s_c) {
      constexpr int S = decltype(s_c)::value;
      if constexpr (S + 2 < 16) issue(std::integral_constant<int, S + 2>{});
      run_step(wave + 4 * (S / 8), std::integral_constant<int, (S % 8) / 2>{}, S & 1, soff[S % 3], std::integral_constant<int, S % 3>{});
    };
    issue(std::integral_constant<int, 0>{});
    issue(std::integral_constant<int, 1>{});
#define UPW_STEP(S_) do_step(std::integral_constant<int, S_>{});
    UPW_STEP(0) UPW_STEP(1) UPW_STEP(2) UPW_STEP(3) UPW_STEP(4) UPW_STEP(5) UPW_STEP(6) UPW_STEP(7)
    CTVAE_PH(up, 1, 3);
    UPW_STEP(8) UPW_STEP(9) UPW_STEP(10) UPW_STEP(11) UPW_STEP(12) UPW_STEP(13) UPW_STEP(14) UPW_STEP(15)
#undef UPW_STEP
    CTVAE_PH(up, 1, 4);
    __syncthreads();
  }
  bsum += __shfl_xor(bsum, 32, 64);
  if (lh == 0) sB[wave * C + li] = bsum;
  auto merge_tap = [&](int wtap, const f32x16& v) {
    __syncthreads();
#pragma unroll
    for (int r = 0; r < 16; ++r) sR[(wave * C + 8 * (r >> 2) + 4 * lh + (r & 3)) * C + li] = v[r];
    __syncthreads();
    for (int e = tid; e < C * C; e += 256) {
      const float s4 = ((sR[e] + sR[C * C + e]) + sR[2 * C * C + e]) + sR[3 * C * C + e];
      a.out[((long)blockIdx.x * NT + wtap) * C * C + e] = s4;
    }
  };
  merge_tap(a.twt[0][0], acc[0]);
  merge_tap(a.twt[1][0], acc[1]);
  merge_tap(a.twt[1][1], acc[2]);
  merge_tap(a.twt[2][0], acc[3]);
  merge_tap(a.twt[2][1], acc[4]);
  merge_tap(a.twt[3][0], acc[5]);
  merge_tap(a.twt[3][1], acc[6]);
  merge_tap(a.twt[3][2], acc[7]);
  merge_tap(a.twt[3][3], acc[8]);
  if (a.pbias != nullptr && tid < C) a.pbias[(long)blockIdx.x * C + tid] = ((sB[tid] + sB[C + tid]) + sB[2 * C + tid]) + sB[3 * C + tid];
  CTVAE_PH(up, 1, 5);
}

void fill(UpArgs& a, const ConvGeom& g) {
  a.B = g.B; a.H = g.gH; a.W = g.gW;
  a.tiles_y = g.gH / TH; a.tiles_x = g.gW / TW;
  a.ntiles = g.B * a.tiles_y * a.tiles_x;
  for (int c = 0; c < NCLS; ++c) {
    a.ntaps[c] = g.ntaps[c]; a.cpy[c] = g.py[c]; a.cpx[c] = g.px[c];
    for (int t = 0; t < MAXT; ++t) {
      const bool ok = t < g.ntaps[c];
      a.tdy[c][t] = ok ? g.taps[c][t].dy : 0;
      a.tdx[c][t] = ok ? g.taps[c][t].dx : 0;
      a.twt[c][t] = ok ? g.taps[c][t].wtap : 0;
    }
  }
}

constexpr size_t kUpFwdSmem = (size_t)(NP * LDA + NT * C * C) * 4;

}

bool upconv_supported(const ConvGeom& g) {
  if (!packed_weights(g) || g.wT != 0 || g.gC != C || g.sC != C || g.wCi != C || g.wCo != C) return false;
  if (g.is != 1 || g.os != 2 || g.ncls != NCLS) return false;
  if (g.sH != 2 * g.gH || g.sW != 2 * g.gW || g.gH % TH != 0 || g.gW % TW != 0) return false;
  int total = 0;
  for (int c = 0; c < NCLS; ++c) {
    if (g.ntaps[c] < 1 || g.ntaps[c] > MAXT) return false;
    total += g.ntaps[c];
    for (int t = 0; t < g.ntaps[c]; ++t) {
      const Tap& tp = g.taps[c][t];
      if (tp.dy < 0 || tp.dy > 1 || tp.dx < 0 || tp.dx > 1 || tp.wtap < 0 || tp.wtap >= NT) return false;
    }
  }
  if (g.ntaps[0] != 1 || g.ntaps[1] != 2 || g.ntaps[2] != 2 || g.ntaps[3] != 4) return false;
  return total == NT && (long)g.B * g.sH * g.sW * C < (1L << 29);
}
bool upconv_wgrad_supported(const ConvGeom& g) { return upconv_supported(g); }

constexpr int kUpWgs = 512;
int upconv_rows(const ConvGeom& g) {
  const int nt = g.B * (g.gH / TH) * (g.gW / TW);
  return nt < kUpWgs ? nt : kUpWgs;
}

int launch_upconv_forward(const ConvGeom& g, const float* X, const float* W, const float* bias, float* S, int act,
                          float* bn_part, hipStream_t st, const InXform* xf) {
  UpArgs a{};
  fill(a, g);
  a.X = X; a.Wt = W; a.bias = bias; a.out = S; a.act = act; a.bn_part = bn_part;
  if (xf != nullptr && xf->scale != nullptr) {
    if (xf->act != ACT_NONE && xf->act != ACT_RELU && xf->act != ACT_LRELU) return kErrBadArg;
    a.xf_scale = xf->scale; a.xf_shift = xf->shift; a.xf_act = xf->act;
  }
  static bool attr_set = false;
  if (!attr_set) {
    (void)hipFuncSetAttribute(reinterpret_cast<const void*>(up_fwd_kernel), hipFuncAttributeMaxDynamicSharedMemorySize, (int)kUpFwdSmem);
    attr_set = true;
  }
  ProfScope ps("up_fwd_kernel", st, 2.0 * a.ntiles * TH * TW * NT * C * C, 4.0 * a.ntiles * TH * TW * C * 5.0);
  hipLaunchKernelGGL(up_fwd_kernel, dim3(upconv_rows(g)), dim3(256), kUpFwdSmem, st, a);
  CTVAE_LAUNCH_CHECK();
  return 0;
}

int launch_upconv_wgrad(const ConvGeom& g, const float* X, const float* dY, float* ws, float** part_out, float** pbias_out,
                        int* nparts, bool want_bias, hipStream_t st, const DyXform* dyx, const InXform* xf) {
  UpArgs a{};
  fill(a, g);
  a.X = X; a.dY = dY;
  if (xf != nullptr && xf->scale != nullptr) {
    if (xf->act != ACT_NONE && xf->act != ACT_RELU && xf->act != ACT_LRELU) return kErrBadArg;
    a.xf_scale = xf->scale; a.xf_shift = xf->shift; a.xf_act = xf->act;
  }
  if (dyx != nullptr && dyx->y != nullptr && dyx->act != ACT_NONE && dyx->act != ACT_RELU && dyx->act != ACT_LRELU) return kErrBadArg;
  if (dyx != nullptr && dyx->y != nullptr) { a.dy_y = dyx->y; a.dy_coef = dyx->coef; a.gy_out = dyx->gy_out; a.dy_act = dyx->act; }
  const int nwg = upconv_rows(g);
  a.out = ws;
  a.pbias = want_bias ? ws + (size_t)nwg * NT * C * C : nullptr;
  ProfScope ps("up_wgrad_kernel", st, 2.0 * a.ntiles * TH * TW * NT * C * C, 4.0 * a.ntiles * TH * TW * C * 5.0);
  if (a.dy_y != nullptr) hipLaunchKernelGGL(up_wgrad_kernel<true>, dim3(nwg), dim3(256), 0, st, a);
  else hipLaunchKernelGGL(up_wgrad_kernel<false>, dim3(nwg), dim3(256), 0, st, a);
  CTVAE_LAUNCH_CHECK();
  *part_out = a.out;
  *pbias_out = a.pbias;
  *nparts = nwg;
  return 0;
}

}
```

ct-vae_amd/native.py:

```python
import ctypes
import os

import torch

_HERE = os.path.dirname(os.path.abspath(__file__))
LIB_PATH = os.environ.get("CTVAE_LIB_OVERRIDE") or os.path.join(_HERE, "lib", "libctvae_hip.so")

_c = ctypes
_fp, _vp, _i, _l, _f, _sz = _c.c_void_p, _c.c_void_p, _c.c_int, _c.c_long, _c.c_float, _c.c_size_t

SIGNATURES = {
    "ctvae_linear_pixmajor_supported": [_i, _i, _i, _i, _sz],
    "ctvae_linear_pixmajor_forward": [_fp, _fp, _fp, _fp, _i, _i, _i, _i, _i, _fp, _sz, _vp],
    "ctvae_conv_forward": [_i, _fp, _fp, _fp, _fp, _fp] + [_i] * 10 + [_fp, _fp, _i, _fp, _fp, _fp, _sz, _vp],
    "ctvae_wino_filters_batch": [_i, _vp, _vp, _vp, _vp, _vp, _vp],
    "ctvae_conv_bn_act_forward": [_i, _fp, _fp, _fp, _fp, _fp, _fp, _fp, _f, _f, _i, _i, _fp, _fp, _fp, _fp, _fp, _fp] + [_i] * 9
                                 + [_fp, _fp, _i, _fp, _sz, _vp],
    "ctvae_conv_dgrad": [_i, _fp, _fp, _fp, _fp, _i, _fp] + [_i] * 9 + [_fp, _fp, _sz, _vp],
    "ctvae_conv_wgrad": [_i, _fp, _fp, _fp, _fp] + [_i] * 10 + [_fp, _fp, _i, _fp, _fp, _i, _fp, _fp, _fp, _i, _fp, _sz, _vp],
    "ctvae_conv_backward": [_i, _fp, _fp, _fp, _fp, _fp, _fp] + [_i] * 10 + [_fp, _i, _fp, _fp, _fp, _fp, _fp, _fp, _i, _fp, _i,
                            _fp, _fp, _fp, _i, _fp, _fp, _i, _fp, _fp, _i, _fp, _fp, _sz, _vp],
    "ctvae_conv_backward_lazy": [_i, _fp, _fp, _fp, _fp, _fp, _fp] + [_i] * 10 + [_fp, _fp, _i, _i, _fp, _sz, _vp],
    "ctvae_bn_backward_fused": [_fp, _i] + [_i] * 10 + [_fp, _fp, _fp, _fp, _fp, _i, _fp, _fp, _fp, _i, _vp],
    "ctvae_bn_forward": [_fp, _i, _i, _fp, _fp, _fp, _fp, _f, _f, _i, _i, _fp, _fp, _fp, _fp, _fp, _sz, _vp],
    "ctvae_bn_backward": [_fp, _fp, _fp, _i, _i, _fp, _fp, _fp, _i, _fp, _fp, _fp, _i, _fp, _i, _fp, _fp, _fp, _sz, _vp],
    "ctvae_permute": [_fp, _fp, _i, _i, _i, _i, _vp],
    "ctvae_crop_resize_u8": [_fp, _fp, _fp, _i, _i, _i, _i, _i, _i, _vp],
    "ctvae_gat_score": [_i, _fp, _fp, _fp, _fp, _fp, _fp, _i, _i, _i, _i, _f, _vp],
    "ctvae_gat_score_backward": [_fp, _fp, _fp, _fp, _fp, _fp, _fp, _fp, _fp, _fp, _i, _i, _i, _i, _f, _vp],
    "ctvae_gat_layer_forward": [_fp, _fp, _i, _fp, _fp, _fp, _fp, _fp, _fp, _i, _fp, _i, _i, _i, _f, _i, _vp],
    "ctvae_gat_layer_backward": [_fp, _fp, _i, _fp, _fp, _fp, _fp, _fp, _fp, _i, _fp, _fp, _fp, _fp, _fp, _fp, _i, _fp, _fp, _fp,
                                 _fp, _i, _i, _i, _i, _f, _i, _vp],
    "ctvae_ct_reg_forward": [_fp, _fp, _fp, _fp, _f, _f, _f, _i, _i, _vp],
    "ctvae_ct_reg_backward": [_fp, _fp, _fp, _fp, _fp, _f, _f, _f, _fp, _fp, _i, _i, _vp],
    "ctvae_ct_blend_softmax_forward": [_fp, _fp, _fp, _l, _i, _i, _vp],
    "ctvae_ct_blend_softmax_backward": [_fp, _fp, _fp, _fp, _fp, _fp, _l, _i, _i, _vp],
    "ctvae_ct_latent_ce_forward": [_fp, _fp, _fp, _l, _i, _vp],
    "ctvae_ct_latent_ce_backward": [_fp, _fp, _fp, _fp, _l, _i, _vp],
    "ctvae_ct_mask_forward": [_fp, _fp, _fp, _fp, _f, _fp, _fp, _fp, _i, _i, _i, _i, _fp, _fp, _fp, _fp, _vp],
    "ctvae_ct_mask_backward": [_fp, _fp, _fp, _fp, _f, _fp, _fp, _fp, _fp, _i, _i, _i, _i, _fp, _fp, _vp],
    "ctvae_ct_blend_forward": [_fp, _fp, _fp, _fp, _l, _vp],
    "ctvae_ct_blend_backward": [_fp, _fp, _fp, _fp, _fp, _fp, _fp, _l, _vp],
    "ctvae_ct_posenc_forward": [_fp, _fp, _fp, _f, _fp, _l, _i, _vp],
    "ctvae_ct_posenc_backward": [_fp, _fp, _f, _fp, _l, _vp],
    "ctvae_one_hot": [_fp, _l, _i, _fp, _vp],
    "ctvae_group_rowsum": [_fp, _l, _i, _i, _i, _i, _fp, _i, _fp, _i, _vp],
    "ctvae_ct_sample_forward": [_fp, _fp, _fp, _fp, _fp, _l, _vp],
    "ctvae_ct_sample_backward": [_fp, _fp, _fp, _fp, _fp, _fp, _l, _vp],
    "ctvae_glinear_forward": [_fp, _i, _i, _i, _i, _vp, _vp, _vp, _vp, _vp, _vp, _fp, _i, _i, _vp],
    "ctvae_glinear_dgrad": [_fp, _i, _i, _i, _vp, _vp, _vp, _vp, _fp, _i, _i, _i, _vp],
    "ctvae_glinear_wgrad": [_fp, _i, _i, _fp, _i, _i, _i, _fp, _i, _i, _fp, _i, _fp, _i, _fp, _sz, _vp],
    "ctvae_pair_mlp_forward": [_fp, _fp, _i, _fp, _fp, _fp, _i, _i, _i, _f, _i, _fp, _vp],
    "ctvae_pair_mlp_backward": [_fp, _fp, _i, _fp, _fp, _fp, _fp, _fp, _i, _fp, _fp, _i, _i, _i, _f, _i, _fp, _vp],
    "ctvae_act_forward": [_fp, _fp, _l, _i, _vp],
    "ctvae_act_backward": [_fp, _fp, _fp, _l, _i, _vp],
    "ctvae_gauss_latent_forward": [_fp, _fp, _fp, _fp, _fp, _i, _i, _fp, _i, _fp, _vp],
    "ctvae_gauss_latent_backward": [_fp, _fp, _fp, _fp, _fp, _fp, _fp, _i, _i, _i, _vp],
    "ctvae_conv_forward_lazy": [_i, _fp, _fp, _fp] + [_i] * 9 + [_fp, _sz, _vp],
    "ctvae_splitk_permute": [_fp, _i, _fp, _i, _i, _i, _vp],
    "ctvae_reparam_forward": [_fp, _l, _fp, _l, _fp, _fp, _i, _i, _vp],
    "ctvae_reparam_backward": [_fp, _fp, _l, _fp, _fp, _fp, _i, _i, _vp],
    "ctvae_loss_forward": [_fp, _fp, _l, _fp, _l, _fp, _l, _i, _i, _f, _fp, _fp, _fp, _sz, _vp],
    "ctvae_loss_forward_grad": [_fp, _fp, _l, _fp, _l, _fp, _l, _i, _i, _f, _fp, _fp, _fp, _fp, _fp, _i, _fp, _sz, _vp],
    "ctvae_mse_backward": [_fp, _fp, _fp, _fp, _l, _i, _vp],
    "ctvae_logcosh_loss_forward": [_fp, _fp, _l, _f, _fp, _l, _fp, _l, _i, _i, _f, _fp, _fp, _sz, _vp],
    "ctvae_logcosh_backward": [_fp, _fp, _fp, _fp, _l, _f, _i, _vp],
    "ctvae_loss_backward": [_fp, _fp, _fp, _fp, _l, _f, _fp, _l, _fp, _l, _fp, _fp, _i, _i, _f, _i, _vp],
    "ctvae_kl_backward": [_fp, _l, _fp, _l, _fp, _fp, _fp, _i, _i, _f, _vp],
    "ctvae_vq_inds": [_fp, _fp, _fp, _i, _i, _i, _i, _i, _vp],
    "ctvae_vq_lookup": [_fp, _fp, _fp, _fp, _fp, _f, _i, _i, _i, _i, _i, _fp, _sz, _vp],
    "ctvae_vq_backward": [_fp, _fp, _fp, _fp, _fp, _fp, _fp, _i, _f, _i, _i, _i, _i, _i, _fp, _sz, _vp],
    "ctvae_gumbel_st_forward": [_fp, _fp, _fp, _fp, _l, _vp],
    "ctvae_gumbel_st_backward": [_fp, _fp, _fp, _fp, _l, _vp],
    "ctvae_gumbel_softmax_forward": [_fp, _fp, _fp, _l, _i, _f, _f, _vp],
    "ctvae_gumbel_softmax_backward": [_fp, _fp, _fp, _l, _i, _f, _vp],
    "ctvae_cat_kl_forward": [_fp, _l, _i, _i, _f, _f, _fp, _fp, _sz, _vp],
    "ctvae_cat_kl_backward": [_fp, _fp, _fp, _l, _i, _i, _f, _f, _vp],
    "ctvae_iw_loss_forward": [_fp, _fp, _l, _i, _i, _fp, _fp, _i, _i, _f, _fp, _fp, _fp, _fp, _vp],
    "ctvae_iw_loss_backward": [_fp, _fp, _l, _i, _i, _fp, _fp, _i, _f, _fp, _fp, _fp, _fp, _fp, _vp],
    "ctvae_l2l1_loss_forward": [_fp, _fp, _l, _fp, _fp, _fp, _sz, _vp],
    "ctvae_l2l1_backward": [_fp, _fp, _fp, _fp, _l, _i, _vp],
    "ctvae_ladder_merge_forward": [_fp, _fp, _fp, _fp, _fp, _i, _i, _fp, _fp, _vp],
    "ctvae_ladder_merge_backward": [_fp, _fp, _fp, _fp, _fp, _fp, _fp, _i, _i, _fp, _fp, _fp, _fp, _vp],
    "ctvae_gamma_reparam_forward": [_fp, _fp, _fp, _f, _fp, _l, _vp],
    "ctvae_gamma_reparam_backward": [_fp, _fp, _fp, _fp, _f, _fp, _fp, _l, _vp],
    "ctvae_gamma_kl_forward": [_fp, _fp, _i, _i, _f, _f, _fp, _fp, _sz, _vp],
    "ctvae_gamma_kl_backward": [_fp, _fp, _fp, _i, _i, _f, _f, _fp, _fp, _vp],
    "ctvae_sigmoid_forward": [_fp, _fp, _l, _vp],
    "ctvae_sigmoid_backward": [_fp, _fp, _fp, _l, _vp],
    "ctvae_tc_forward": [_fp, _fp, _fp, _fp, _i, _i, _fp, _fp, _fp, _fp, _sz, _vp],
    "ctvae_tc_backward": [_fp, _fp, _fp, _fp, _fp, _fp, _fp, _i, _i, _fp, _fp, _fp, _vp],
    "ctvae_vamp_kl_forward": [_fp, _fp, _fp, _fp, _fp, _i, _i, _i, _fp, _fp, _fp, _sz, _vp],
    "ctvae_vamp_kl_backward": [_fp, _fp, _fp, _fp, _fp, _fp, _fp, _i, _i, _i, _fp, _fp, _fp, _fp, _fp, _vp],
    "ctvae_swd_forward": [_fp, _fp, _fp, _i, _i, _i, _f, _f, _fp, _fp, _fp, _sz, _vp],
    "ctvae_mmd_forward": [_fp, _fp, _i, _i, _i, _f, _f, _f, _f, _f, _fp, _fp, _fp, _sz, _vp],
    "ctvae_dip_forward": [_fp, _l, _fp, _l, _i, _i, _f, _f, _fp, _vp],
    "ctvae_dip_backward": [_fp, _fp, _fp, _fp, _i, _i, _vp],
    "ctvae_column_moments": [_fp, _i, _i, _fp, _fp, _fp, _fp, _vp],
    "ctvae_mi_matrix": [_fp, _fp, _fp, _fp, _fp, _i, _i, _i, _fp, _fp, _vp],
    "ctvae_group_var_argmin": [_fp, _fp, _fp, _i, _i, _i, _fp, _fp, _vp],
    "ctvae_image_grid_u8": [_fp, _l, _l, _l, _l, _i, _i, _i, _i, _i, _i, _i, _i, _f, _f, _f, _i, _fp, _sz, _fp, _sz, _vp],
    "ctvae_image_grid_each_u8": [_fp, _l, _l, _l, _l, _i, _i, _i, _i, _i, _i, _i, _i, _f, _f, _f, _i, _fp, _sz, _fp, _sz, _vp],
    "ctvae_action_hits": [_fp, _fp, _i, _i, _fp, _vp],
    "ctvae_adam_step": [_fp, _fp, _fp, _fp, _fp, _l, _f, _vp],
    "ctvae_adam_step_clipped": [_fp, _fp, _fp, _fp, _fp, _l, _f, _i, _f, _fp, _fp, _vp],
    "ctvae_adam_mark_members": [_fp, _i, _fp, _i, _vp],
    "ctvae_adam_block_flags": [_fp, _fp, _fp, _i, _fp, _fp, _i, _i, _vp],
    "ctvae_adam_block_flags_local": [_fp, _fp, _fp, _i, _fp, _i, _vp],
    "ctvae_adam_block_flags_finish": [_fp, _fp, _i, _i, _vp],
    "ctvae_adam_step_blocks": [_fp, _fp, _fp, _fp, _fp, _l, _f, _i, _f, _fp, _fp, _fp, _fp, _fp, _fp, _i, _vp],
    "ctvae_mssim_forward": [_fp, _fp, _fp, _fp, _fp, _fp, _fp, _i, _i, _i, _i, _vp],
    "ctvae_mssim_backward": [_fp, _fp, _fp, _fp, _fp, _fp, _i, _i, _i, _i, _vp],
    "ctvae_defer_begin": [_fp, _sz],
    "ctvae_defer_flush": [_vp],
}
_RESTYPES = {
    "ctvae_version": _c.c_char_p,
    "ctvae_arch": _c.c_char_p,
    "ctvae_error_string": _c.c_char_p,
    "ctvae_workspace_bytes": _c.c_size_t,
    "ctvae_prof_enable": None,
    "ctvae_prof_calibrate": None,
    "ctvae_prof_report": _c.c_size_t,
    "ctvae_conv_backward_bn_rows": _c.c_int,
    "ctvae_conv_backward_lazy_slices": _c.c_int,
    "ctvae_conv_forward_lazy_slices": _c.c_int,
    "ctvae_conv_bn_act_apply_is_separate": _c.c_int,
    "ctvae_winograd_enable": _c.c_int,
    "ctvae_conv_wino_filter_floats": _c.c_size_t,
    "ctvae_dip_state_floats": _c.c_size_t,
    "ctvae_adam_state_floats": _c.c_size_t,
    "ctvae_grad_clip_workspace_floats": _c.c_size_t,
    "ctvae_mssim_part_floats": _c.c_size_t,
    "ctvae_glinear_wgrad_ws_bytes": _c.c_size_t,
    "ctvae_conv_input_transform_supported": _c.c_int,
    "ctvae_conv_wgrad_bn_apply_supported": _c.c_int,
}
EXPORTS = sorted(list(SIGNATURES) + list(_RESTYPES))

_lib = None


def load():
    global _lib
    if _lib is not None:
        return _lib
    if not os.path.exists(LIB_PATH):
        raise RuntimeError(
            f"{LIB_PATH} is missing: build it with `python -m ctvae_amd.build` (hipcc, gfx950). "
            "There is no CPU/PyTorch fallback for the ctvae hot path.")
    try:
        lib = ctypes.CDLL(LIB_PATH)
    except OSError as e:
        raise RuntimeError(f"cannot load {LIB_PATH}: {e}") from e
    for name, argtypes in SIGNATURES.items():
        fn = getattr(lib, name, None)
        if fn is None:
            raise RuntimeError(f"{LIB_PATH} does not export {name} (stale build?)")
        fn.argtypes = argtypes
        fn.restype = _c.c_int
    for name, res in _RESTYPES.items():
        fn = getattr(lib, name, None)
        if fn is None:
            raise RuntimeError(f"{LIB_PATH} does not export {name} (stale build?)")
        fn.restype = res
        fn.argtypes = {"ctvae_error_string": [_c.c_int], "ctvae_prof_enable": [_c.c_int],
                       "ctvae_prof_calibrate": [_c.c_void_p, _c.c_int],
                       "ctvae_prof_report": [_c.c_char_p, _c.c_size_t],
                       "ctvae_conv_backward_bn_rows": [_c.c_int] * 10 + [_c.c_size_t],
                       "ctvae_conv_backward_lazy_slices": [_c.c_int] * 11 + [_c.c_size_t],
                       "ctvae_conv_forward_lazy_slices": [_c.c_int] * 10 + [_c.c_size_t],
                       "ctvae_conv_bn_act_apply_is_separate": [_c.c_int] * 10 + [_c.c_size_t],
                       "ctvae_winograd_enable": [_c.c_int],
                       "ctvae_dip_state_floats": [_c.c_int, _c.c_int],
                       "ctvae_glinear_wgrad_ws_bytes": [_c.c_int] * 5,
                       "ctvae_conv_wino_filter_floats": [_c.c_int] * 10 + [_c.c_size_t],
                       "ctvae_conv_input_transform_supported": [_c.c_int] * 10,
                       "ctvae_conv_wgrad_bn_apply_supported": [_c.c_int] * 10}.get(name, [])
    if lib.ctvae_arch() != b"gfx950":
        raise RuntimeError("libctvae_hip.so was not built for gfx950")
    _lib = lib
    return lib


def check(code: int, what: str):
    if code != 0:
        msg = load().ctvae_error_string(int(code)).decode()
        raise RuntimeError(f"{what} failed: {msg} (code {code})")


def stream_ptr() -> int:
    return torch.cuda.current_stream().cuda_stream


def ptr(t):
    return None if t is None else t.data_ptr()


_workspaces = {}


def workspace(device) -> torch.Tensor:
    key = (device.index if device.index is not None else torch.cuda.current_device(), torch.cuda.current_stream().cuda_stream)
    ws = _workspaces.get(key)
    if ws is None:
        n = load().ctvae_workspace_bytes()
        ws = torch.empty(n // 4, dtype=torch.float32, device=device)
        _workspaces[key] = ws
    return ws


def call(name: str, *args):
    lib = load()
    check(getattr(lib, name)(*args, stream_ptr()), name)


_wino_on = None


def winograd_enable(on: bool) -> bool:
    global _wino_on
    prev = bool(load().ctvae_winograd_enable(1 if on else 0))
    _wino_on = bool(on)
    return prev


def winograd_enabled() -> bool:
    global _wino_on
    if _wino_on is None:
        lib = load()
        _wino_on = bool(lib.ctvae_winograd_enable(1))
        lib.ctvae_winograd_enable(1 if _wino_on else 0)
    return _wino_on


def prof_enable(on, detailed: bool = False):
    load().ctvae_prof_enable((2 if detailed else 1) if on else 0)


def prof_calibrate(n: int = 64):
    load().ctvae_prof_calibrate(stream_ptr(), n)


def prof_report() -> dict:
    lib = load()
    buf = ctypes.create_string_buffer(1 << 16)
    lib.ctvae_prof_report(buf, len(buf))
    out = {}
    for line in buf.value.decode().splitlines():
        name, cnt, ms, fl, by = line.split("\t")
        out[name] = dict(count=int(cnt), ms=float(ms), flops=float(fl), bytes=float(by))
    return out
```

include/ctvae_hip.h:

```cpp
#ifndef CTVAE_HIP_H
#define CTVAE_HIP_H
#include <stddef.h>
#include <stdint.h>

#ifdef __cplusplus
extern "C" {
#endif

#define CTVAE_ACT_NONE 0
#define CTVAE_ACT_LRELU 1
#define CTVAE_ACT_RELU 2
#define CTVAE_ACT_TANH 3

#define CTVAE_CONV 0
#define CTVAE_CONVT 1
#define CTVAE_W_CI_TAP 0x100

const char* ctvae_version(void);
const char* ctvae_arch(void);
const char* ctvae_error_string(int code);
size_t ctvae_workspace_bytes(void);

int ctvae_conv_forward(int kind, const float* x, const float* w, const float* bias, const float* add, float* y, int B,
                       int H, int W, int Ci, int Co, int k, int stride, int pad, int out_pad, int act, const float* in_scale,
                       const float* in_shift, int in_act, float* wino_dgrad_filters_out, const float* wino_fwd_filters, float* ws,
                       size_t ws_bytes, void* stream);
int ctvae_linear_pixmajor_supported(int B, int Ci, int C, int P, size_t ws_bytes);
int ctvae_linear_pixmajor_forward(const float* x, const float* w, const float* bias, float* y, int B, int Ci, int C, int P, int act,
                                  float* ws, size_t ws_bytes, void* stream);
int ctvae_wino_filters_batch(int n, const float* const* w, float* const* fwd_filters, float* const* dgrad_filters, const int* Ci,
                             const int* Co, void* stream);
size_t ctvae_conv_wino_filter_floats(int kind, int B, int H, int W, int Ci, int Co, int k, int stride, int pad, int out_pad,
                                     size_t ws_bytes);
int ctvae_conv_input_transform_supported(int kind, int B, int H, int W, int Ci, int Co, int k, int stride, int pad,
                                         int out_pad);

int ctvae_conv_bn_act_apply_is_separate(int kind, int B, int H, int W, int Ci, int Co, int k, int stride, int pad, int out_pad,
                                        size_t ws_bytes);
int ctvae_conv_bn_act_forward(int kind, const float* x, const float* w, const float* bias, const float* gamma,
                              const float* beta, float* running_mean, float* running_var, float momentum, float eps,
                              int training, int act, float* y, float* a_out, float* save_mean, float* save_invstd,
                              float* scale_shift_out, int64_t* num_batches_tracked, int B, int H, int W, int Ci, int Co, int k,
                              int stride, int pad, int out_pad, const float* in_scale, const float* in_shift, int in_act,
                              float* ws, size_t ws_bytes, void* stream);

int ctvae_conv_dgrad(int kind, const float* dy, const float* w, const float* add, const float* mask, int mask_act,
                     float* dx, int B, int H, int W, int Ci, int Co, int k, int stride, int pad, int out_pad,
                     const float* wino_filters, float* ws, size_t ws_bytes, void* stream);

int ctvae_conv_wgrad(int kind, const float* x, const float* dy, float* dw, float* dbias, int B, int H, int W, int Ci,
                     int Co, int k, int stride, int pad, int out_pad, int accumulate, const float* in_scale,
                     const float* in_shift, int in_act, const float* dy_bn_y, const float* dy_bn_coef, int dy_bn_act,
                     float* gy_out, float* bn_dgamma, float* bn_dbeta, int bn_accumulate, float* ws, size_t ws_bytes,
                     void* stream);
int ctvae_conv_backward_bn_rows(int kind, int B, int H, int W, int Ci, int Co, int k, int stride, int pad, int out_pad,
                                size_t ws_bytes);
int ctvae_conv_backward(int kind, const float* x, const float* dy, const float* w, float* dw, float* dbias, float* dx, int B,
                        int H, int W, int Ci, int Co, int k, int stride, int pad, int out_pad, int accumulate, const float* mask,
                        int mask_act, const float* wino_filters, const float* bn_y, const float* bn_mean,
                        const float* bn_invstd, const float* bn_gamma, const float* bn_beta, int bn_act, float* bn_part,
                        int bn_part_rows, float* bn_coef_out, float* bn_dgamma, float* bn_dbeta, int bn_accumulate,
                        const float* in_scale, const float* in_shift, int in_act,
                        const float* dy_bn_y, const float* dy_bn_coef, int dy_bn_act, float* gy_out, float* ws, size_t ws_bytes,
                        void* stream);

int ctvae_conv_backward_lazy_slices(int kind, int B, int H, int W, int Ci, int Co, int k, int stride, int pad, int out_pad,
                                    int for_bn, size_t ws_bytes);
int ctvae_conv_backward_lazy(int kind, const float* x, const float* dy, const float* w, float* dw, float* dbias, float* dx_slices,
                             int B, int H, int W, int Ci, int Co, int k, int stride, int pad, int out_pad, int accumulate,
                             const float* in_scale, const float* in_shift, int in_act, int pixel_major, float* ws, size_t ws_bytes,
                             void* stream);
int ctvae_bn_backward_fused(const float* g_a_slices, int slices, int kind, int B, int H, int W, int Ci, int Co, int k, int stride,
                            int pad, int out_pad, const float* y, const float* gamma, const float* beta, const float* save_mean,
                            const float* save_invstd, int act, float* g_y, float* dgamma, float* dbeta, int accumulate, void* stream);

int ctvae_conv_wgrad_bn_apply_supported(int kind, int B, int H, int W, int Ci, int Co, int k, int stride, int pad,
                                        int out_pad);

int ctvae_bn_forward(const float* y, int R, int C, const float* gamma, const float* beta, float* running_mean,
                     float* running_var, float momentum, float eps, int training, int act, float* out,
                     float* save_mean, float* save_invstd, int64_t* num_batches_tracked, float* ws, size_t ws_bytes,
                     void* stream);
int ctvae_bn_backward(const float* g_a, const float* beta, const float* y, int R, int C, const float* gamma,
                      const float* save_mean, const float* save_invstd, int act, float* g_y, float* dgamma,
                      float* dbeta, int accumulate, const float* part_in, int part_rows, float* coef_out,
                      const float* coef_in, float* ws, size_t ws_bytes, void* stream);

int ctvae_pair_mlp_forward(const float* u, const float* v, int ld, const float* w2, const float* b2, float* out, int B, int N,
                           int H, float slope, int per_sample, const int32_t* row_of, void* stream);
int ctvae_pair_mlp_backward(const float* u, const float* v, int ld, const float* w2, const float* out, const float* g_out,
                            float* d_u, float* d_v, int ldd, float* d_w2_part, float* d_b2_part, int B, int N, int H, float slope,
                            int per_sample, const int32_t* row_of, void* stream);

int ctvae_gat_score(int mode, const float* xl, const float* xr, const float* attr, const float* we, const float* att, float* out,
                    int B, int N, int H, int C, float slope, void* stream);
int ctvae_gat_score_backward(const float* xl, const float* xr, const float* attr, const float* we, const float* att,
                             const float* g, float* d_xl, float* d_xr, float* d_att_part, float* d_we_part, int B, int N, int H,
                             int C, float slope, void* stream);

int ctvae_gat_layer_forward(const float* xl, const float* xr, int ld, const float* adj, const float* we, const float* att,
                            const float* bias, const int32_t* head_map, float* out, int ldo, float* alpha, int B, int Hs, int C,
                            float slope, int act, void* stream);
int ctvae_gat_layer_backward(const float* xl, const float* xr, int ld, const float* adj, const float* we, const float* att,
                             const float* bias, const int32_t* head_map, const float* out, int ldo, const float* alpha,
                             const float* g_out, float* dS, float* dattr, float* d_xl, float* d_xr, int ldd, float* d_bias_part,
                             float* d_att_part, float* d_we_part, float* d_adj, int accumulate_dadj, int B, int Hs, int C,
                             float slope, int act, void* stream);

int ctvae_glinear_forward(const float* x, int ldx, int K, int nseg, int N, const float* const* W, const int* ldw,
                          const int64_t* w_gstride, const float* const* bias, const int* b_gstride,
                          const int32_t* const* group, float* y, int ldy, int B, void* stream);
int ctvae_glinear_dgrad(const float* dy, int ldy, int nseg, int N, const float* const* W, const int* ldw,
                        const int64_t* w_gstride, const int32_t* const* group, float* dx, int ldx, int K, int B, void* stream);
size_t ctvae_glinear_wgrad_ws_bytes(int G, int N, int K, int B, int grouped);
int ctvae_glinear_wgrad(const float* x, int ldx, int K, const float* dy, int ldy, int col0, int N, const int32_t* group, int G,
                        int B, float* dW, int ldo, float* dbias, int accumulate, float* ws, size_t ws_bytes, void* stream);

int ctvae_ct_blend_forward(const float* s0, const float* s1, const float* mask, float* out, long rows, void* stream);
int ctvae_ct_blend_backward(const float* g, const float* s0, const float* s1, const float* mask, float* g0, float* g1, float* g_mask,
                            long rows, void* stream);
int ctvae_ct_posenc_forward(const float* x, const float* pe, const float* keep, float scale, float* out, long n, int sd,
                            void* stream);
int ctvae_ct_posenc_backward(const float* g, const float* keep, float scale, float* g_x, long n, void* stream);
int ctvae_one_hot(const int64_t* inds, long n, int N, float* out, void* stream);
int ctvae_group_rowsum(const float* parts, long mat_stride, int nmat, int rows, int C, int ld, const int32_t* group, int G, float* out,
                       int accumulate, void* stream);

int ctvae_ct_reg_forward(const float* adj, const float* graph, const float* uniform, float* part4, float ckl, float cgs, float cpt,
                         int B, int N, void* stream);
int ctvae_ct_reg_backward(const float* adj, const float* graph, const float* uniform, const float* part4, const float* g_loss,
                          float ckl, float cgs, float cpt, float* d_adj, float* d_graph, int B, int N, void* stream);
int ctvae_ct_blend_softmax_forward(const float* y, const float* mask, float* probs, long R, int Hs, int D, void* stream);
int ctvae_ct_blend_softmax_backward(const float* g, const float* probs, const float* y, const float* mask, float* dy, float* dmask,
                                    long R, int Hs, int D, void* stream);
int ctvae_ct_latent_ce_forward(const float* probs, const int64_t* target, float* row_loss, long R, int D, void* stream);
int ctvae_ct_latent_ce_backward(const float* probs, const int64_t* target, const float* g_loss, float* d_probs, long R, int D,
                                void* stream);

int ctvae_ct_mask_forward(const float* x, const float* action, const float* pe, const float* keep, float scale, const float* W,
                          const float* bias, const float* expo, int B, int S, int D, int A, float* inter, float* p, float* sample,
                          float* soft, void* stream);
int ctvae_ct_mask_backward(const float* x, const float* action, const float* pe, const float* keep, float scale, const float* inter,
                           const float* p, const float* soft, const float* g, int B, int S, int D, int A, float* dWp, float* dbp,
                           void* stream);
int ctvae_ct_sample_forward(const float* p, const float* expo, float* sample, float* soft, float* weighted, long n, void* stream);
int ctvae_ct_sample_backward(const float* g_sample, const float* g_weighted, const float* p, const float* soft, const float* sample,
                             float* g_p, long n, void* stream);

int ctvae_permute(const float* in, float* out, int B, int C, int P, int to_nhwc, void* stream);
int ctvae_act_forward(const float* in, float* out, long n, int act, void* stream);
int ctvae_act_backward(const float* g_out, const float* out, float* g_in, long n, int act, void* stream);

int ctvae_gauss_latent_forward(float* heads, const float* eps_in, const uint64_t* rng, float* eps_out, float* z, int B, int L,
                               const float* head_slices, int slices, const float* head_bias, void* stream);
int ctvae_gauss_latent_backward(const float* g_mu, const float* g_logvar, const float* g_z, const float* heads, const float* eps,
                                float* g_heads, uint64_t* rng_bump, int B, int L, int g_z_slices, void* stream);
int ctvae_conv_forward_lazy_slices(int kind, int B, int H, int W, int Ci, int Co, int k, int stride, int pad, int out_pad,
                                   size_t ws_bytes);
int ctvae_conv_forward_lazy(int kind, const float* x, const float* w, float* y_slices, int B, int H, int W, int Ci, int Co, int k,
                            int stride, int pad, int out_pad, float* ws, size_t ws_bytes, void* stream);
int ctvae_splitk_permute(const float* slices, int n_slices, float* out, int B, int C, int P, void* stream);
int ctvae_reparam_forward(const float* mu, long mu_row_stride, const float* logvar, long lv_row_stride, const float* eps,
                          float* z, int B, int L, void* stream);
int ctvae_reparam_backward(const float* g_z, const float* logvar, long lv_row_stride, const float* eps, float* g_mu,
                           float* g_logvar, int B, int L, void* stream);

int ctvae_loss_forward(const float* recons, const float* x, long n, const float* mu, long mu_row_stride,
                       const float* logvar, long lv_row_stride, int B, int L, float M_N, const float* extra, float* out4,
                       float* ws, size_t ws_bytes, void* stream);
int ctvae_loss_forward_grad(const float* recons, const float* x, long n, const float* mu, long mu_row_stride, const float* logvar,
                            long lv_row_stride, int B, int L, float M_N, const float* extra, float* out4, float* g_recons,
                            float* g_mu, float* g_logvar, int recons_act, float* ws, size_t ws_bytes, void* stream);
int ctvae_mse_backward(const float* recons, const float* x, const float* g_loss, float* g_recons, long n, int recons_act,
                       void* stream);
int ctvae_loss_backward(const float* recons, const float* x, const float* g_loss, float* g_recons, long n, float logcosh_alpha,
                        const float* mu, long mu_row_stride, const float* logvar, long lv_row_stride, float* g_mu, float* g_logvar,
                        int B, int L, float M_N, int recons_act, void* stream);
int ctvae_logcosh_loss_forward(const float* recons, const float* x, long n, float alpha, const float* mu, long mu_row_stride,
                               const float* logvar, long lv_row_stride, int B, int L, float M_N, float* out4, float* ws,
                               size_t ws_bytes, void* stream);
int ctvae_logcosh_backward(const float* recons, const float* x, const float* g_loss, float* g_recons, long n, float alpha,
                           int recons_act, void* stream);
int ctvae_kl_backward(const float* mu, long mu_row_stride, const float* logvar, long lv_row_stride, const float* g_loss,
                      float* g_mu, float* g_logvar, int B, int L, float M_N, void* stream);

int ctvae_vq_inds(const float* latents, const float* codebooks, int64_t* inds, int B, int HW, int D, int K, int C,
                  void* stream);
int ctvae_vq_lookup(const float* latents, const float* codebooks, const int64_t* inds, float* quantized, float* vq_loss,
                    float beta, int B, int HW, int D, int K, int C, float* ws, size_t ws_bytes, void* stream);
int ctvae_vq_backward(const float* g_quantized, const float* g_vq_loss, const float* latents, const float* codebooks,
                      const int64_t* inds, float* g_latents, float* d_codebooks, int accumulate, float beta, int B, int HW,
                      int D, int K, int C, float* ws, size_t ws_bytes, void* stream);

int ctvae_gumbel_st_forward(const float* p, const float* gumbel_noise, float* sample, float* soft, long n, void* stream);
int ctvae_gumbel_st_backward(const float* g_sample, const float* p, const float* soft, float* g_p, long n, void* stream);

int ctvae_gumbel_softmax_forward(const float* logits, const float* uniform, float* sample, long rows, int Q, float temperature,
                                 float eps, void* stream);
int ctvae_gumbel_softmax_backward(const float* g_sample, const float* sample, float* g_logits, long rows, int Q,
                                  float temperature, void* stream);
int ctvae_cat_kl_forward(const float* logits, long rows, int Q, int B, float eps, float log_prior, float* kld, float* ws,
                         size_t ws_bytes, void* stream);
int ctvae_cat_kl_backward(const float* logits, const float* g_kld, float* g_logits, long rows, int Q, int B, float eps,
                          float log_prior, void* stream);

int ctvae_iw_loss_forward(const float* recons, const float* x, long n, int R, int rep, const float* mu, const float* logvar,
                          int L, int S, float M_N, float* lp, float* kld, float* coef, float* out4, void* stream);
int ctvae_iw_loss_backward(const float* recons, const float* x, long n, int R, int rep, const float* mu, const float* logvar,
                           int L, float M_N, const float* coef, const float* g_loss, float* g_recons, float* g_mu,
                           float* g_logvar, void* stream);

int ctvae_l2l1_loss_forward(const float* recons, const float* x, long n, const float* extra, float* out4, float* ws, size_t ws_bytes,
                            void* stream);
int ctvae_l2l1_backward(const float* recons, const float* x, const float* g_loss, float* g_recons, long n, int recons_act,
                        void* stream);
int ctvae_ladder_merge_forward(const float* mu_e, const float* logvar_e, const float* mu_t, const float* logvar_t, const float* eps,
                               int B, int D, float* z, float* kl, void* stream);
int ctvae_ladder_merge_backward(const float* g_z, const float* g_kl, const float* mu_e, const float* logvar_e, const float* mu_t,
                                const float* logvar_t, const float* eps, int B, int D, float* g_mu_e, float* g_logvar_e,
                                float* g_mu_t, float* g_logvar_t, void* stream);
int ctvae_gamma_reparam_forward(const float* alpha, const float* beta, const float* zhat, float gamma_shape, float* z, long n,
                                void* stream);
int ctvae_gamma_reparam_backward(const float* g_z, const float* alpha, const float* beta, const float* zhat, float gamma_shape,
                                 float* g_alpha, float* g_beta, long n, void* stream);
int ctvae_gamma_kl_forward(const float* alpha, const float* beta, int B, int D, float prior_alpha, float prior_beta, float* out,
                           float* ws, size_t ws_bytes, void* stream);
int ctvae_gamma_kl_backward(const float* g_kld, const float* alpha, const float* beta, int B, int D, float prior_alpha,
                            float prior_beta, float* g_alpha, float* g_beta, void* stream);
int ctvae_sigmoid_forward(const float* x, float* y, long n, void* stream);
int ctvae_sigmoid_backward(const float* g, const float* y, float* g_x, long n, void* stream);
int ctvae_tc_forward(const float* z, const float* mu, const float* logvar, const float* log_iw, int B, int D, float* out3, float* lse_s,
                     float* lse_d, float* ws, size_t ws_bytes, void* stream);
int ctvae_tc_backward(const float* z, const float* mu, const float* logvar, const float* log_iw, const float* lse_s, const float* lse_d,
                      const float* g3, int B, int D, float* g_z, float* g_mu, float* g_logvar, void* stream);
int ctvae_vamp_kl_forward(const float* z, const float* mu, const float* logvar, const float* prior_mu, const float* prior_logvar,
                          int B, int D, int K, float* out3, float* weights, float* ws, size_t ws_bytes, void* stream);
int ctvae_vamp_kl_backward(const float* z, const float* mu, const float* logvar, const float* prior_mu, const float* prior_logvar,
                           const float* weights, const float* g_kld, int B, int D, int K, float* g_z, float* g_mu, float* g_logvar,
                           float* g_prior_mu, float* g_prior_logvar, void* stream);
int ctvae_swd_forward(const float* z, const float* prior, const float* proj, int N, int D, int S, float p, float weight, float* out,
                      float* grad_z, float* ws, size_t ws_bytes, void* stream);

int ctvae_mmd_forward(const float* z, const float* prior, int N, int D, int kind, float c, float eps, float w_pp, float w_zz,
                      float w_pz, float* out4, float* grad_z, float* ws, size_t ws_bytes, void* stream);

size_t ctvae_dip_state_floats(int B, int D);
int ctvae_dip_forward(const float* mu, long mu_row_stride, const float* logvar, long lv_row_stride, int B, int D,
                      float lambda_diag, float lambda_offdiag, float* state, void* stream);
int ctvae_dip_backward(const float* state, const float* g_dip, float* g_mu, float* g_logvar, int B, int D, void* stream);

int ctvae_column_moments(const float* z, int N, int L, float* mean, float* var, float* min, float* max, void* stream);
int ctvae_mi_matrix(const float* z, const float* lo, const float* hi, const int32_t* factors, const int32_t* sizes, int N, int L,
                    int F, float* mi, uint8_t* bins, void* stream);
int ctvae_group_var_argmin(const float* z, const float* global_var, const uint8_t* active, int G, int B, int L, int32_t* arg,
                           float* val, void* stream);

int ctvae_image_grid_u8(const float* x, long stride_n, long stride_c, long stride_h, long stride_w, int N, int C, int H, int W,
                        int nrow, int padding, int normalize, int has_range, float range_lo, float range_hi, float pad_value,
                        int scanlines, uint8_t* out, size_t out_bytes, float* workspace, size_t workspace_bytes, void* stream);

int ctvae_image_grid_each_u8(const float* x, long stride_n, long stride_c, long stride_h, long stride_w, int N, int C, int H, int W,
                             int nrow, int padding, int normalize, int has_range, float range_lo, float range_hi, float pad_value,
                             int scanlines, uint8_t* out, size_t out_bytes, float* workspace, size_t workspace_bytes, void* stream);

int ctvae_action_hits(const float* probas, const float* action, int N, int A, int* counts, void* stream);

size_t ctvae_mssim_part_floats(int B, int C);
int ctvae_mssim_forward(const float* a, const float* b, const float* window, const float* weights, float* part, float* loss,
                        float* coef, int B, int C, int H, int W, void* stream);
int ctvae_mssim_backward(const float* a, const float* b, const float* window, const float* coef, const float* g_loss, float* g_a,
                         int B, int C, int H, int W, void* stream);

int ctvae_defer_begin(float* arena, size_t arena_bytes);
int ctvae_defer_flush(void* stream);

size_t ctvae_adam_state_floats(void);
int ctvae_adam_step(float* params, const float* grads, float* exp_avg, float* exp_avg_sq, float* state, long n,
                    float grad_scale, void* stream);

#define CTVAE_CLIP_NORM 0
#define CTVAE_CLIP_VALUE 1
size_t ctvae_grad_clip_workspace_floats(void);
int ctvae_adam_step_clipped(float* params, const float* grads, float* exp_avg, float* exp_avg_sq, float* state, long n,
                            float grad_scale, int algorithm, float clip_val, float* workspace, float* norm_out, void* stream);

#define CTVAE_ADAM_NO_CLIP 2
int ctvae_adam_mark_members(int* hits, int nhits, const int* group, int B, void* stream);
int ctvae_adam_block_flags(const int* present, const int* hit_index, int* hits, int nhits, const float* block_state, int* active,
                           int nb, int until_first, void* stream);
int ctvae_adam_block_flags_local(const int* present, const int* hit_index, int* hits, int nhits, int* active, int nb, void* stream);
int ctvae_adam_block_flags_finish(const float* block_state, int* active, int nb, int until_first, void* stream);
int ctvae_adam_step_blocks(float* params, const float* grads, float* exp_avg, float* exp_avg_sq, float* state, long n,
                           float grad_scale, int algorithm, float clip_val, float* workspace, float* norm_out,
                           const int* block_lo, const int* block_hi, float* block_state, const int* active, int nb, void* stream);

int ctvae_crop_resize_u8(const uint8_t* images, const int64_t* rows, float* out, int B, int N, int H, int W, int crop, int size,
                         void* stream);

int ctvae_winograd_enable(int on);

void ctvae_prof_enable(int on);
void ctvae_prof_calibrate(void* stream, int n);
size_t ctvae_prof_report(char* buf, size_t n);

#ifdef __cplusplus
}
#endif
#endif
```

Baseline: 88700 images/s.

## Add 8-wave upconv forward and wgrad kernels for small tile counts

Adds 512-thread (8-wave) variants of the transposed-conv forward and weight-gradient kernels, used when the number of output tiles is at most 256. In the forward kernel each wave handles one output row instead of two. In the wgrad kernel one tile goes to each workgroup: one 4-wave group computes the four-tap class while the other computes the remaining classes, and the partial results are merged through LDS. The aim is more parallelism and shorter per-workgroup critical paths when the grid is too small to fill the GPU. The cost is higher register and LDS pressure per workgroup, and the wgrad path requires the workgroup count to equal the tile count.

```diff
diff --git a/ct-vae_amd/csrc/api.hip b/ct-vae_amd/csrc/api.hip
--- a/ct-vae_amd/csrc/api.hip
+++ b/ct-vae_amd/csrc/api.hip
@@ -39,6 +39,7 @@
 int launch_wino_filters_batch(int n, const float* const* W, float* const* Uf, float* const* Ub, const int* Ci, const int* Co,
                               hipStream_t st);
 bool upconv_wgrad_supported(const ConvGeom& g);
+int upconv_wg_waves_of(int B, int H, int W);
 bool img_enc_supported(const ConvGeom& g);
 bool img_conv_supported(const ConvGeom& g);
 int launch_img_backward_fused(const ConvGeom& g, const float* dY, const float* W, float* dX, const BnBwdFuse* bnb, float* ws,
@@ -532,6 +533,8 @@
   return img_enc_supported(g) ? 2 : 0;
 }
 
+int ctvae_upconv_wg_waves(int B, int H, int W) { return upconv_wg_waves_of(B, H, W); }
+
 int ctvae_bn_forward(const float* y, int R, int C, const float* gamma, const float* beta, float* running_mean,
                      float* running_var, float momentum, float eps, int training, int act, float* out,
                      float* save_mean, float* save_invstd, int64_t* num_batches_tracked, float* ws, size_t ws_bytes,
diff --git a/ct-vae_amd/csrc/upconv.hip b/ct-vae_amd/csrc/upconv.hip
--- a/ct-vae_amd/csrc/upconv.hip
+++ b/ct-vae_amd/csrc/upconv.hip
@@ -10,7 +10,7 @@
 
 constexpr int TH = 8, TW = 32, PH = 9, PW = 33, NP = PH * PW ;
 constexpr int LDA = 36, C = 32, NT = 9, NCLS = 4, MAXT = 4;
-constexpr int NLD = (NP * 8 + 255) / 256;
+constexpr int nld(int nthr) { return (NP * 8 + nthr - 1) / nthr; }
 constexpr unsigned kOOBu = 0x80000000u;
 
 struct UpArgs {
@@ -57,13 +57,15 @@
   return TileXY{b, ty * TH, (r - ty * a.tiles_x) * TW};
 }
 
+template <int NTHR>
 struct Patch {
-  f32x4 v[NLD];
-};
-__device__ __forceinline__ void patch_load(const UpArgs& a, __amdgpu_buffer_rsrc_t rX, const TileXY& t, Patch& p) {
-#pragma unroll
-  for (int j = 0; j < NLD; ++j) {
-    const int e = threadIdx.x + 256 * j;
+  f32x4 v[nld(NTHR)];
+};
+template <int NTHR>
+__device__ __forceinline__ void patch_load(const UpArgs& a, __amdgpu_buffer_rsrc_t rX, const TileXY& t, Patch<NTHR>& p) {
+#pragma unroll
+  for (int j = 0; j < nld(NTHR); ++j) {
+    const int e = threadIdx.x + NTHR * j;
     const int pp = e >> 3, c4 = e & 7;
     const int py = (pp * 1986) >> 16, px = pp - py * PW;
     const int iy = t.y0 + py, ix = t.x0 + px;
@@ -71,18 +73,20 @@
     p.v[j] = ld4(rX, ok ? (unsigned)(((t.b * a.H + iy) * a.W + ix) * C + 4 * c4) * 4u : kOOBu);
   }
 }
-__device__ __forceinline__ void patch_store(const Patch& p, float* sA) {
-#pragma unroll
-  for (int j = 0; j < NLD; ++j) {
-    const int e = threadIdx.x + 256 * j;
+template <int NTHR>
+__device__ __forceinline__ void patch_store(const Patch<NTHR>& p, float* sA) {
+#pragma unroll
+  for (int j = 0; j < nld(NTHR); ++j) {
+    const int e = threadIdx.x + NTHR * j;
     if (e < NP * 8) *reinterpret_cast<f32x4*>(&sA[(e >> 3) * LDA + 4 * (e & 7)]) = p.v[j];
   }
 }
-__device__ __forceinline__ void patch_store_xf(const UpArgs& a, const TileXY& t, const Patch& p, float* sA, f32x4 sc, f32x4 sh,
+template <int NTHR>
+__device__ __forceinline__ void patch_store_xf(const UpArgs& a, const TileXY& t, const Patch<NTHR>& p, float* sA, f32x4 sc, f32x4 sh,
                                                float nslope) {
 #pragma unroll
-  for (int j = 0; j < NLD; ++j) {
-    const int e = threadIdx.x + 256 * j;
+  for (int j = 0; j < nld(NTHR); ++j) {
+    const int e = threadIdx.x + NTHR * j;
     const int pp = e >> 3;
     const int py = (pp * 1986) >> 16, px = pp - py * PW;
     const float inside = (t.y0 + py < a.H && t.x0 + px < a.W) ? 1.f : 0.f;
@@ -97,24 +101,28 @@
 }
 
 CTVAE_PHASE_DECL(up)
-__global__ __launch_bounds__(256, 2) void up_fwd_kernel(const UpArgs a) {
+template <int NW>
+__device__ __forceinline__ void up_fwd_body(const UpArgs& a) {
+  constexpr int NTHR = 64 * NW;
+  static_assert(TH % NW == 0, "whole rows per wave");
   CTVAE_PH(up, 0, 0);
   kernarg_warm<sizeof(UpArgs)>();
   extern __shared__ __attribute__((aligned(16))) float smem[];
   float* sA = smem;
   float* sW = smem + NP * LDA;
-  __shared__ float sS[4 * C * 3];
+  __shared__ float sS[NW * C * 3];
   const int tid = threadIdx.x, lane = tid & 63, wave = tid >> 6, li = lane & 31, lh = lane >> 5;
   const __amdgpu_buffer_rsrc_t rX = rsrc(a.X, (long)a.B * a.H * a.W * C * 4);
   const int OH = 2 * a.H, OW = 2 * a.W;
   const __amdgpu_buffer_rsrc_t rO = rsrc(a.out, (long)a.B * OH * OW * C * 4);
 
-  constexpr int NW4 = NT * C * C / 4 / 256;
-  static_assert(NW4 * 256 * 4 == NT * C * C, "weights: a whole number of 16-byte loads per thread");
+  constexpr int NWQ = NT * C * C / 4, NW4 = (NWQ + NTHR - 1) / NTHR;
+  constexpr bool kWholeW = NWQ % NTHR == 0;
   f32x4 wv[NW4];
 #pragma unroll
-  for (int j = 0; j < NW4; ++j) wv[j] = reinterpret_cast<const f32x4*>(a.Wt)[tid + 256 * j];
-  Patch pt;
+  for (int j = 0; j < NW4; ++j)
+    if (kWholeW || tid + NTHR * j < NWQ) wv[j] = reinterpret_cast<const f32x4*>(a.Wt)[tid + NTHR * j];
+  Patch<NTHR> pt;
   int tile = blockIdx.x;
   TileXY cur = tile_xy(a, tile < a.ntiles ? tile : 0);
   if (tile < a.ntiles) patch_load(a, rX, cur, pt);
@@ -127,7 +135,8 @@
   const f32x4 xsh = xf ? *reinterpret_cast<const f32x4*>(a.xf_shift + 4 * (tid & 7)) : f32x4{0.f, 0.f, 0.f, 0.f};
   const float xns = a.xf_act == ACT_LRELU ? kLeaky : (a.xf_act == ACT_RELU ? 0.f : 1.f);
 #pragma unroll
-  for (int j = 0; j < NW4; ++j) reinterpret_cast<f32x4*>(sW)[tid + 256 * j] = wv[j];
+  for (int j = 0; j < NW4; ++j)
+    if (kWholeW || tid + NTHR * j < NWQ) reinterpret_cast<f32x4*>(sW)[tid + NTHR * j] = wv[j];
   for (; tile < a.ntiles; tile += gridDim.x) {
     CTVAE_PH(up, 0, 1);
     if (xf) patch_store_xf(a, cur, pt, sA, xsc, xsh, xns);
@@ -200,8 +209,8 @@
     __builtin_amdgcn_sched_barrier(0);
     Frag fa, fb;
 #pragma unroll 1
-    for (int i = 0; i < 2; ++i) {
-      const int ly = wave + 4 * i;
+    for (int i = 0; i < TH / NW; ++i) {
+      const int ly = wave + NW * i;
       f32x16 acc;
       read_tap(ly, 0, 0, fa);
       zero(acc);
@@ -247,7 +256,7 @@
     if (tid < C) {
       float n = 0.f, mean = 0.f, m2 = 0.f;
 #pragma unroll
-      for (int w = 0; w < 4; ++w) {
+      for (int w = 0; w < NW; ++w) {
         const float nb = sS[(w * C + tid) * 3], mb = sS[(w * C + tid) * 3 + 1], qb = sS[(w * C + tid) * 3 + 2];
         if (nb > 0.f) {
           const float ntot = n + nb, d = mb - mean;
@@ -262,12 +271,160 @@
   }
 }
 
+__global__ __launch_bounds__(256, 2) void up_fwd_kernel(const UpArgs a) { up_fwd_body<4>(a); }
+__global__ __launch_bounds__(512, 2) void up8_fwd_kernel(const UpArgs a) { up_fwd_body<8>(a); }
 
 template <int CLS>
 struct ClsInfo {
   static constexpr int ntaps = CLS == 0 ? 1 : (CLS == 3 ? 4 : 2);
   static constexpr int first = CLS == 0 ? 0 : (CLS == 1 ? 1 : (CLS == 2 ? 3 : 5));
 };
+
+struct SchedAll {
+  static constexpr int nsteps = 16, nacc = NT;
+  static constexpr int row(int s) { return s / 8; }
+  static constexpr int cls(int s) { return (s % 8) / 2; }
+  static constexpr int first(int c) { return c == 0 ? 0 : (c == 1 ? 1 : (c == 2 ? 3 : 5)); }
+};
+struct SchedC3 {
+  static constexpr int nsteps = 4, nacc = 4;
+  static constexpr int row(int s) { return s / 2; }
+  static constexpr int cls(int) { return 3; }
+  static constexpr int first(int) { return 0; }
+};
+struct SchedC012 {
+  static constexpr int nsteps = 12, nacc = 5;
+  static constexpr int row(int s) { return s / 6; }
+  static constexpr int cls(int s) { return (s % 6) / 2; }
+  static constexpr int first(int c) { return c == 0 ? 0 : (c == 1 ? 1 : 3); }
+};
+
+template <int S, int N, class F>
+__device__ __forceinline__ void static_for(F&& f) {
+  if constexpr (S < N) {
+    f(std::integral_constant<int, S>{});
+    static_for<S + 1, N>(f);
+  }
+}
+
+template <int NTHR, int J0, int NJ>
+__device__ __forceinline__ void stage_patch(const UpArgs& a, __amdgpu_buffer_rsrc_t rX, const TileXY& cur, float* sA, bool xf, f32x4 xsc,
+                                            f32x4 xsh, float xns) {
+  const int tid = threadIdx.x;
+  f32x4 v[NJ];
+#pragma unroll
+  for (int j = 0; j < NJ; ++j) {
+    const int e = tid + NTHR * (j + J0);
+    const int pp = e >> 3, c4 = e & 7;
+    const int py = (pp * 1986) >> 16, px = pp - py * PW;
+    const int iy = cur.y0 + py, ix = cur.x0 + px;
+    const bool ok = e < NP * 8 && iy < a.H && ix < a.W;
+    v[j] = ld4(rX, ok ? (unsigned)(((cur.b * a.H + iy) * a.W + ix) * C + 4 * c4) * 4u : kOOBu);
+  }
+  if (xf) {
+#pragma unroll
+    for (int j = 0; j < NJ; ++j) {
+      const int e = tid + NTHR * (j + J0);
+      const int pp = e >> 3;
+      const int py = (pp * 1986) >> 16, px = pp - py * PW;
+      const float inside = (cur.y0 + py < a.H && cur.x0 + px < a.W) ? 1.f : 0.f;
+#pragma unroll
+      for (int q = 0; q < 4; ++q) {
+        const float u = v[j][q] * xsc[q] + xsh[q] * inside;
+        v[j][q] = fmaxf(u, u * xns);
+      }
+    }
+  }
+#pragma unroll
+  for (int j = 0; j < NJ; ++j) {
+    const int e = tid + NTHR * (j + J0);
+    if (e < NP * 8) *reinterpret_cast<f32x4*>(&sA[(e >> 3) * LDA + 4 * (e & 7)]) = v[j];
+  }
+}
+
+struct DyCoef {
+  float k1, k2, k3, ksc, ksh, nslope;
+};
+template <bool FUSED>
+__device__ __forceinline__ DyCoef dy_coef(const UpArgs& a, int li) {
+  DyCoef k;
+  k.k1 = FUSED ? a.dy_coef[li] : 0.f; k.k2 = FUSED ? a.dy_coef[C + li] : 0.f; k.k3 = FUSED ? a.dy_coef[2 * C + li] : 0.f;
+  k.ksc = FUSED ? a.dy_coef[3 * C + li] : 0.f; k.ksh = FUSED ? a.dy_coef[4 * C + li] : 0.f;
+  k.nslope = a.dy_act == ACT_LRELU ? kLeaky : (a.dy_act == ACT_RELU ? 0.f : 1.f);
+  return k;
+}
+
+template <bool FUSED, class SCHED, int NACC>
+__device__ __forceinline__ void wgrad_tile_steps(const UpArgs& a, const TileXY& cur, const float* sA, __amdgpu_buffer_rsrc_t rG,
+                                                 __amdgpu_buffer_rsrc_t rYb, __amdgpu_buffer_rsrc_t rGY, const DyCoef& k, int wrow, int li,
+                                                 int lh, f32x16 (&acc)[NACC], float& bsum) {
+  static_assert(SCHED::nacc <= NACC, "accumulators of the schedule");
+  const int OH = 2 * a.H, OW = 2 * a.W;
+  float dv[3][8], yv[FUSED ? 3 : 1][FUSED ? 8 : 1];
+  auto step_off = [&](int ly, int c, int h) {
+    return (unsigned)((((cur.b * OH + 2 * (cur.y0 + ly) + a.cpy[c]) * OW + 2 * cur.x0 + a.cpx[c] + 2 * (16 * h + lh)) * C + li)) * 4u;
+  };
+  auto dy_load = [&](unsigned off, auto slot_c) {
+    constexpr int slot = decltype(slot_c)::value;
+#pragma unroll
+    for (int j = 0; j < 8; ++j) dv[slot][j] = ld1(rG, off + (unsigned)(4 * j * C) * 4u);
+    if constexpr (FUSED) {
+#pragma unroll
+      for (int j = 0; j < 8; ++j) yv[slot][j] = ld1(rYb, off + (unsigned)(4 * j * C) * 4u);
+    }
+  };
+  auto run_step = [&](int ly, auto cls_c, int h, unsigned off, auto slot_c) {
+    constexpr int CLS = decltype(cls_c)::value;
+    constexpr int slot = decltype(slot_c)::value;
+    constexpr int first = SCHED::first(CLS);
+    using CI = ClsInfo<CLS>;
+    int xo[CI::ntaps];
+#pragma unroll
+    for (int t = 0; t < CI::ntaps; ++t) xo[t] = ((ly + a.tdy[CLS][t]) * PW + 16 * h + lh + a.tdx[CLS][t]) * LDA + li;
+    float xa[CI::ntaps], xb[CI::ntaps];
+#pragma unroll
+    for (int t = 0; t < CI::ntaps; ++t) xa[t] = sA[xo[t]];
+#pragma unroll
+    for (int j = 0; j < 8; ++j) {
+      if (j + 1 < 8) {
+#pragma unroll
+        for (int t = 0; t < CI::ntaps; ++t) xb[t] = sA[xo[t] + 2 * (j + 1) * LDA];
+      }
+      float d = dv[slot][j];
+      if constexpr (FUSED) {
+        const float yy = yv[slot][j];
+        const float g1 = (yy * k.ksc + k.ksh) > 0.f ? d : d * k.nslope;
+        d = k.k1 * g1 + k.k2 * yy + k.k3;
+        st1(rGY, off + (unsigned)(4 * j * C) * 4u, d);
+      }
+      bsum += d;
+#pragma unroll
+      for (int t = 0; t < CI::ntaps; ++t)
+        acc[first + t] = __builtin_amdgcn_mfma_f32_32x32x2f32(xa[t], d, acc[first + t], 0, 0, 0);
+#pragma unroll
+      for (int t = 0; t < CI::ntaps; ++t) xa[t] = xb[t];
+      __builtin_amdgcn_sched_barrier(0);
+    }
+  };
+  unsigned soff[3];
+  auto issue = [&](auto s_c) {
+    constexpr int S = decltype(s_c)::value;
+    soff[S % 3] = step_off(wrow + 4 * SCHED::row(S), SCHED::cls(S), S & 1);
+    dy_load(soff[S % 3], std::integral_constant<int, S % 3>{});
+  };
+  issue(std::integral_constant<int, 0>{});
+  issue(std::integral_constant<int, 1>{});
+  static_for<0, SCHED::nsteps>([&](auto s_c) {
+    constexpr int S = decltype(s_c)::value;
+    if constexpr (S + 2 < SCHED::nsteps) issue(std::integral_constant<int, S + 2>{});
+    run_step(wrow + 4 * SCHED::row(S), std::integral_constant<int, SCHED::cls(S)>{}, S & 1, soff[S % 3], std::integral_constant<int, S % 3>{});
+  });
+}
+
+__device__ __forceinline__ void acc_to_lds(float* dst, const f32x16& v, int li, int lh) {
+#pragma unroll
+  for (int r = 0; r < 16; ++r) dst[(8 * (r >> 2) + 4 * lh + (r & 3)) * C + li] = v[r];
+}
 
 template <bool FUSED>
 __global__ __launch_bounds__(256, 1) void up_wgrad_kernel(const UpArgs a) {
@@ -277,14 +434,11 @@
   __shared__ float sB[4 * C];
   const int tid = threadIdx.x, lane = tid & 63, wave = tid >> 6, li = lane & 31, lh = lane >> 5;
   const __amdgpu_buffer_rsrc_t rX = rsrc(a.X, (long)a.B * a.H * a.W * C * 4);
-  const int OH = 2 * a.H, OW = 2 * a.W;
-  const long obytes = (long)a.B * OH * OW * C * 4;
+  const long obytes = (long)a.B * 2 * a.H * 2 * a.W * C * 4;
   const __amdgpu_buffer_rsrc_t rG = rsrc(a.dY, obytes);
   const __amdgpu_buffer_rsrc_t rYb = rsrc(a.dy_y, FUSED ? obytes : 0);
   const __amdgpu_buffer_rsrc_t rGY = rsrc(a.gy_out, FUSED ? obytes : 0);
-  const float k1 = FUSED ? a.dy_coef[li] : 0.f, k2 = FUSED ? a.dy_coef[C + li] : 0.f, k3 = FUSED ? a.dy_coef[2 * C + li] : 0.f;
-  const float ksc = FUSED ? a.dy_coef[3 * C + li] : 0.f, ksh = FUSED ? a.dy_coef[4 * C + li] : 0.f;
-  const float nslope = a.dy_act == ACT_LRELU ? kLeaky : (a.dy_act == ACT_RELU ? 0.f : 1.f);
+  const DyCoef k = dy_coef<FUSED>(a, li);
   const bool xf = a.xf_scale != nullptr;
   const f32x4 xsc = xf ? *reinterpret_cast<const f32x4*>(a.xf_scale + 4 * (tid & 7)) : f32x4{0.f, 0.f, 0.f, 0.f};
   const f32x4 xsh = xf ? *reinterpret_cast<const f32x4*>(a.xf_shift + 4 * (tid & 7)) : f32x4{0.f, 0.f, 0.f, 0.f};
@@ -301,113 +455,19 @@
   for (int tile = blockIdx.x; tile < a.ntiles; tile += gridDim.x) {
     const TileXY cur = tile_xy(a, tile);
     CTVAE_PH(up, 1, 1);
-#pragma unroll
-    for (int h = 0; h < 2; ++h) {
-      f32x4 v[NLD / 2];
-#pragma unroll
-      for (int j = 0; j < NLD / 2; ++j) {
-        const int e = tid + 256 * (j + h * (NLD / 2));
-        const int pp = e >> 3, c4 = e & 7;
-        const int py = (pp * 1986) >> 16, px = pp - py * PW;
-        const int iy = cur.y0 + py, ix = cur.x0 + px;
-        const bool ok = e < NP * 8 && iy < a.H && ix < a.W;
-        v[j] = ld4(rX, ok ? (unsigned)(((cur.b * a.H + iy) * a.W + ix) * C + 4 * c4) * 4u : kOOBu);
-      }
-      if (xf) {
-#pragma unroll
-        for (int j = 0; j < NLD / 2; ++j) {
-          const int e = tid + 256 * (j + h * (NLD / 2));
-          const int pp = e >> 3;
-          const int py = (pp * 1986) >> 16, px = pp - py * PW;
-          const float inside = (cur.y0 + py < a.H && cur.x0 + px < a.W) ? 1.f : 0.f;
-#pragma unroll
-          for (int q = 0; q < 4; ++q) {
-            const float u = v[j][q] * xsc[q] + xsh[q] * inside;
-            v[j][q] = fmaxf(u, u * xns);
-          }
-        }
-      }
-#pragma unroll
-      for (int j = 0; j < NLD / 2; ++j) {
-        const int e = tid + 256 * (j + h * (NLD / 2));
-        if (e < NP * 8) *reinterpret_cast<f32x4*>(&sA[(e >> 3) * LDA + 4 * (e & 7)]) = v[j];
-      }
-    }
-    __syncthreads();
-
+    stage_patch<256, 0, nld(256) / 2>(a, rX, cur, sA, xf, xsc, xsh, xns);
+    stage_patch<256, nld(256) / 2, nld(256) / 2>(a, rX, cur, sA, xf, xsc, xsh, xns);
+    __syncthreads();
     CTVAE_PH(up, 1, 2);
-    float dv[3][8], yv[FUSED ? 3 : 1][FUSED ? 8 : 1];
-    auto step_off = [&](int ly, int c, int h) {
-      return (unsigned)((((cur.b * OH + 2 * (cur.y0 + ly) + a.cpy[c]) * OW + 2 * cur.x0 + a.cpx[c] + 2 * (16 * h + lh)) * C + li)) * 4u;
-    };
-    auto dy_load = [&](unsigned off, auto slot_c) {
-      constexpr int slot = decltype(slot_c)::value;
-#pragma unroll
-      for (int j = 0; j < 8; ++j) dv[slot][j] = ld1(rG, off + (unsigned)(4 * j * C) * 4u);
-      if constexpr (FUSED) {
-#pragma unroll
-        for (int j = 0; j < 8; ++j) yv[slot][j] = ld1(rYb, off + (unsigned)(4 * j * C) * 4u);
-      }
-    };
-    auto run_step = [&](int ly, auto cls_c, int h, unsigned off, auto slot_c) {
-      constexpr int CLS = decltype(cls_c)::value;
-      constexpr int slot = decltype(slot_c)::value;
-      using CI = ClsInfo<CLS>;
-      int xo[CI::ntaps];
-#pragma unroll
-      for (int t = 0; t < CI::ntaps; ++t) xo[t] = ((ly + a.tdy[CLS][t]) * PW + 16 * h + lh + a.tdx[CLS][t]) * LDA + li;
-      float xa[CI::ntaps], xb[CI::ntaps];
-#pragma unroll
-      for (int t = 0; t < CI::ntaps; ++t) xa[t] = sA[xo[t]];
-#pragma unroll
-      for (int j = 0; j < 8; ++j) {
-        if (j + 1 < 8) {
-#pragma unroll
-          for (int t = 0; t < CI::ntaps; ++t) xb[t] = sA[xo[t] + 2 * (j + 1) * LDA];
-        }
-        float d = dv[slot][j];
-        if constexpr (FUSED) {
-          const float yy = yv[slot][j];
-          const float g1 = (yy * ksc + ksh) > 0.f ? d : d * nslope;
-          d = k1 * g1 + k2 * yy + k3;
-          st1(rGY, off + (unsigned)(4 * j * C) * 4u, d);
-        }
-        bsum += d;
-#pragma unroll
-        for (int t = 0; t < CI::ntaps; ++t)
-          acc[CI::first + t] = __builtin_amdgcn_mfma_f32_32x32x2f32(xa[t], d, acc[CI::first + t], 0, 0, 0);
-#pragma unroll
-        for (int t = 0; t < CI::ntaps; ++t) xa[t] = xb[t];
-        __builtin_amdgcn_sched_barrier(0);
-      }
-    };
-    unsigned soff[3];
-    auto issue = [&](auto s_c) {
-      constexpr int S = decltype(s_c)::value;
-      soff[S % 3] = step_off(wave + 4 * (S / 8), (S % 8) / 2, S & 1);
-      dy_load(soff[S % 3], std::integral_constant<int, S % 3>{});
-    };
-    auto do_step = [&](auto s_c) {
-      constexpr int S = decltype(s_c)::value;
-      if constexpr (S + 2 < 16) issue(std::integral_constant<int, S + 2>{});
-      run_step(wave + 4 * (S / 8), std::integral_constant<int, (S % 8) / 2>{}, S & 1, soff[S % 3], std::integral_constant<int, S % 3>{});
-    };
-    issue(std::integral_constant<int, 0>{});
-    issue(std::integral_constant<int, 1>{});
-#define UPW_STEP(S_) do_step(std::integral_constant<int, S_>{});
-    UPW_STEP(0) UPW_STEP(1) UPW_STEP(2) UPW_STEP(3) UPW_STEP(4) UPW_STEP(5) UPW_STEP(6) UPW_STEP(7)
+    wgrad_tile_steps<FUSED, SchedAll>(a, cur, sA, rG, rYb, rGY, k, wave, li, lh, acc, bsum);
     CTVAE_PH(up, 1, 3);
-    UPW_STEP(8) UPW_STEP(9) UPW_STEP(10) UPW_STEP(11) UPW_STEP(12) UPW_STEP(13) UPW_STEP(14) UPW_STEP(15)
-#undef UPW_STEP
-    CTVAE_PH(up, 1, 4);
     __syncthreads();
   }
   bsum += __shfl_xor(bsum, 32, 64);
   if (lh == 0) sB[wave * C + li] = bsum;
   auto merge_tap = [&](int wtap, const f32x16& v) {
     __syncthreads();
-#pragma unroll
-    for (int r = 0; r < 16; ++r) sR[(wave * C + 8 * (r >> 2) + 4 * lh + (r & 3)) * C + li] = v[r];
+    acc_to_lds(sR + wave * C * C, v, li, lh);
     __syncthreads();
     for (int e = tid; e < C * C; e += 256) {
       const float s4 = ((sR[e] + sR[C * C + e]) + sR[2 * C * C + e]) + sR[3 * C * C + e];
@@ -424,7 +484,75 @@
   merge_tap(a.twt[3][2], acc[7]);
   merge_tap(a.twt[3][3], acc[8]);
   if (a.pbias != nullptr && tid < C) a.pbias[(long)blockIdx.x * C + tid] = ((sB[tid] + sB[C + tid]) + sB[2 * C + tid]) + sB[3 * C + tid];
-  CTVAE_PH(up, 1, 5);
+  CTVAE_PH(up, 1, 4);
+}
+
+template <bool FUSED>
+__global__ __launch_bounds__(512, 2) void up8_wgrad_kernel(const UpArgs a) {
+  kernarg_warm<sizeof(UpArgs)>();
+  __shared__ __attribute__((aligned(16))) float sA[NP * LDA];
+  __shared__ float sB[8 * C];
+  static_assert(8 * C * C <= NP * LDA, "the merge buffer fits the patch");
+  const int tid = threadIdx.x, lane = tid & 63, wave = tid >> 6, li = lane & 31, lh = lane >> 5;
+  const int grp = __builtin_amdgcn_readfirstlane(wave >> 2), wrow = wave & 3;
+  const __amdgpu_buffer_rsrc_t rX = rsrc(a.X, (long)a.B * a.H * a.W * C * 4);
+  const long obytes = (long)a.B * 2 * a.H * 2 * a.W * C * 4;
+  const __amdgpu_buffer_rsrc_t rG = rsrc(a.dY, obytes);
+  const __amdgpu_buffer_rsrc_t rYb = rsrc(a.dy_y, FUSED ? obytes : 0);
+  const __amdgpu_buffer_rsrc_t rGY = rsrc(a.gy_out, FUSED ? obytes : 0);
+  const DyCoef k = dy_coef<FUSED>(a, li);
+  const bool xf = a.xf_scale != nullptr;
+  const f32x4 xsc = xf ? *reinterpret_cast<const f32x4*>(a.xf_scale + 4 * (tid & 7)) : f32x4{0.f, 0.f, 0.f, 0.f};
+  const f32x4 xsh = xf ? *reinterpret_cast<const f32x4*>(a.xf_shift + 4 * (tid & 7)) : f32x4{0.f, 0.f, 0.f, 0.f};
+  const float xns = a.xf_act == ACT_LRELU ? kLeaky : (a.xf_act == ACT_RELU ? 0.f : 1.f);
+
+  constexpr int NA = SchedC012::nacc;
+  f32x16 acc[NA];
+#pragma unroll
+  for (int t = 0; t < NA; ++t)
+#pragma unroll
+    for (int r = 0; r < 16; ++r) acc[t][r] = 0.f;
+  float bsum = 0.f;
+
+  CTVAE_PH(up, 1, 0);
+  const TileXY cur = tile_xy(a, blockIdx.x);
+  CTVAE_PH(up, 1, 1);
+  stage_patch<512, 0, nld(512)>(a, rX, cur, sA, xf, xsc, xsh, xns);
+  __syncthreads();
+  CTVAE_PH(up, 1, 2);
+  if (grp == 0) wgrad_tile_steps<FUSED, SchedC3>(a, cur, sA, rG, rYb, rGY, k, wrow, li, lh, acc, bsum);
+  else wgrad_tile_steps<FUSED, SchedC012>(a, cur, sA, rG, rYb, rGY, k, wrow, li, lh, acc, bsum);
+  CTVAE_PH(up, 1, 3);
+  bsum += __shfl_xor(bsum, 32, 64);
+  if (lh == 0) sB[wave * C + li] = bsum;
+  auto merge_round = [&](int r, int wtap3, int wtap012, const f32x16& v) {
+    __syncthreads();
+    if (grp == 1 || r < SchedC3::nacc) acc_to_lds(sA + wave * C * C, v, li, lh);
+    __syncthreads();
+#pragma unroll
+    for (int h = 0; h < 2; ++h) {
+      if (h == 0 && r >= SchedC3::nacc) continue;
+#pragma unroll
+      for (int q = 0; q < 2; ++q) {
+        const int e = tid + 512 * q;
+        const float* s = sA + h * 4 * C * C + e;
+        const float s4 = ((s[0] + s[C * C]) + s[2 * C * C]) + s[3 * C * C];
+        a.out[((long)blockIdx.x * NT + (h == 0 ? wtap3 : wtap012)) * C * C + e] = s4;
+      }
+    }
+  };
+  merge_round(0, a.twt[3][0], a.twt[0][0], acc[0]);
+  merge_round(1, a.twt[3][1], a.twt[1][0], acc[1]);
+  merge_round(2, a.twt[3][2], a.twt[1][1], acc[2]);
+  merge_round(3, a.twt[3][3], a.twt[2][0], acc[3]);
+  merge_round(4, 0, a.twt[2][1], acc[4]);
+  if (a.pbias != nullptr && tid < C) {
+    float s = sB[tid];
+#pragma unroll
+    for (int w = 1; w < 8; ++w) s += sB[w * C + tid];
+    a.pbias[(long)blockIdx.x * C + tid] = s;
+  }
+  CTVAE_PH(up, 1, 4);
 }
 
 void fill(UpArgs& a, const ConvGeom& g) {
@@ -464,6 +592,14 @@
 }
 bool upconv_wgrad_supported(const ConvGeom& g) { return upconv_supported(g); }
 
+constexpr int kUpOneRound = 256;
+int upconv_wg_waves(int ntiles) { return ntiles <= kUpOneRound ? 8 : 4; }
+int upconv_wg_waves_of(int B, int H, int W) {
+  if (B < 1 || H < TH || W < TW || H % TH != 0 || W % TW != 0) return 0;
+  if ((long)B * (2L * H) * (2L * W) * C >= (1L << 29)) return 0;
+  return upconv_wg_waves(B * (H / TH) * (W / TW));
+}
+
 constexpr int kUpWgs = 512;
 int upconv_rows(const ConvGeom& g) {
   const int nt = g.B * (g.gH / TH) * (g.gW / TW);
@@ -482,10 +618,12 @@
   static bool attr_set = false;
   if (!attr_set) {
     (void)hipFuncSetAttribute(reinterpret_cast<const void*>(up_fwd_kernel), hipFuncAttributeMaxDynamicSharedMemorySize, (int)kUpFwdSmem);
+    (void)hipFuncSetAttribute(reinterpret_cast<const void*>(up8_fwd_kernel), hipFuncAttributeMaxDynamicSharedMemorySize, (int)kUpFwdSmem);
     attr_set = true;
   }
   ProfScope ps("up_fwd_kernel", st, 2.0 * a.ntiles * TH * TW * NT * C * C, 4.0 * a.ntiles * TH * TW * C * 5.0);
-  hipLaunchKernelGGL(up_fwd_kernel, dim3(upconv_rows(g)), dim3(256), kUpFwdSmem, st, a);
+  if (upconv_wg_waves(a.ntiles) == 8) hipLaunchKernelGGL(up8_fwd_kernel, dim3(upconv_rows(g)), dim3(512), kUpFwdSmem, st, a);
+  else hipLaunchKernelGGL(up_fwd_kernel, dim3(upconv_rows(g)), dim3(256), kUpFwdSmem, st, a);
   CTVAE_LAUNCH_CHECK();
   return 0;
 }
@@ -505,8 +643,14 @@
   a.out = ws;
   a.pbias = want_bias ? ws + (size_t)nwg * NT * C * C : nullptr;
   ProfScope ps("up_wgrad_kernel", st, 2.0 * a.ntiles * TH * TW * NT * C * C, 4.0 * a.ntiles * TH * TW * C * 5.0);
-  if (a.dy_y != nullptr) hipLaunchKernelGGL(up_wgrad_kernel<true>, dim3(nwg), dim3(256), 0, st, a);
-  else hipLaunchKernelGGL(up_wgrad_kernel<false>, dim3(nwg), dim3(256), 0, st, a);
+  if (upconv_wg_waves(a.ntiles) == 8) {
+    if (nwg != a.ntiles) return kErrBadArg;
+    if (a.dy_y != nullptr) hipLaunchKernelGGL(up8_wgrad_kernel<true>, dim3(nwg), dim3(512), 0, st, a);
+    else hipLaunchKernelGGL(up8_wgrad_kernel<false>, dim3(nwg), dim3(512), 0, st, a);
+  } else {
+    if (a.dy_y != nullptr) hipLaunchKernelGGL(up_wgrad_kernel<true>, dim3(nwg), dim3(256), 0, st, a);
+    else hipLaunchKernelGGL(up_wgrad_kernel<false>, dim3(nwg), dim3(256), 0, st, a);
+  }
   CTVAE_LAUNCH_CHECK();
   *part_out = a.out;
   *pbias_out = a.pbias;
diff --git a/ct-vae_amd/native.py b/ct-vae_amd/native.py
--- a/ct-vae_amd/native.py
+++ b/ct-vae_amd/native.py
@@ -135,6 +135,7 @@
     "ctvae_glinear_wgrad_ws_bytes": _c.c_size_t,
     "ctvae_conv_input_transform_supported": _c.c_int,
     "ctvae_conv_wgrad_bn_apply_supported": _c.c_int,
+    "ctvae_upconv_wg_waves": _c.c_int,
 }
 EXPORTS = sorted(list(SIGNATURES) + list(_RESTYPES))
 
@@ -176,7 +177,8 @@
                        "ctvae_glinear_wgrad_ws_bytes": [_c.c_int] * 5,
                        "ctvae_conv_wino_filter_floats": [_c.c_int] * 10 + [_c.c_size_t],
                        "ctvae_conv_input_transform_supported": [_c.c_int] * 10,
-                       "ctvae_conv_wgrad_bn_apply_supported": [_c.c_int] * 10}.get(name, [])
+                       "ctvae_conv_wgrad_bn_apply_supported": [_c.c_int] * 10,
+                       "ctvae_upconv_wg_waves": [_c.c_int] * 3}.get(name, [])
     if lib.ctvae_arch() != b"gfx950":
         raise RuntimeError("libctvae_hip.so was not built for gfx950")
     _lib = lib
diff --git a/include/ctvae_hip.h b/include/ctvae_hip.h
--- a/include/ctvae_hip.h
+++ b/include/ctvae_hip.h
@@ -76,6 +76,8 @@
 
 int ctvae_conv_wgrad_bn_apply_supported(int kind, int B, int H, int W, int Ci, int Co, int k, int stride, int pad,
                                         int out_pad);
+
+int ctvae_upconv_wg_waves(int B, int H, int W);
 
 int ctvae_bn_forward(const float* y, int R, int C, const float* gamma, const float* beta, float* running_mean,
                      float* running_var, float momentum, float eps, int training, int act, float* out,
```

New measurement: 89730 images/s, median of 6. +1.2%, better.
